# galuszkm/STAN

Hardware: AMD Instinct MI355X
Metric: DOF/s (assembly+CG to 1e-8) on 10M-DOF HEX8 cube; SpMV GB/s vs HBM peak (higher is better)
Workload: dtype f64

## Files before the change

### include/stan_hip.h

```cpp
#ifndef STAN_HIP_H
#define STAN_HIP_H

#include <stdint.h>

#ifdef __cplusplus
extern "C" {
#endif

typedef struct stan_ctx stan_ctx;
typedef struct stan_matrix stan_matrix;

#define STAN_OK 0
#define STAN_E_HIP (-1)
#define STAN_E_ARG (-2)
#define STAN_E_ALLOC (-3)
#define STAN_E_DETJ (-4)
#define STAN_E_DOF_LAYOUT (-5)
#define STAN_E_VALENCE (-6)
#define STAN_E_COMM (-7)
#define STAN_E_UNSUPPORTED (-8)

#define STAN_HEX8_G1 1
#define STAN_HEX8_G2 2

#define STAN_PREC_FP64 0
#define STAN_PREC_MIXED 1
#define STAN_PREC_FIXED48 2
#define STAN_VALUE_STREAM_60 3

int stan_hip_init(int device, stan_ctx **out);
int stan_hip_init_multi(int n_devices, const int *devices, stan_ctx **out);
void stan_hip_destroy(stan_ctx *ctx);
const char *stan_hip_last_error(stan_ctx *ctx);
int64_t stan_hip_last_bad_element(stan_ctx *ctx);
int stan_hip_set_stream(stan_ctx *ctx, void *hip_stream);

#define STAN_OPT_CG_MERIT_STOP 1
#define STAN_OPT_CG_RUPDATE 2
#define STAN_OPT_OVERLAP_HALO 4
#define STAN_OPT_ASSEMBLY_MODE 5
#define STAN_OPT_CG_FUSED_REFRESH 6
#define STAN_OPT_CG_SINGLE_REDUCE 10
#define STAN_OPT_CG_FOLD_REDUCE 11
#define STAN_OPT_VEC_STORE_NT 12
#define STAN_OPT_PACKED_COLUMNS 13
#define STAN_OPT_CG_DEFER_X 14
#define STAN_OPT_SPMV_SMALL 15
#define STAN_OPT_PLACEMENT_TRIES 8
#define STAN_OPT_PLACEMENT_MAX_BYTES 16
#define STAN_OPT_SELL_SIGMA 17
#define STAN_OPT_ROW_FOLDING 19
#define STAN_OPT_COMM_P2P 18
#define STAN_OPT_CG_REFINE 20
#define STAN_OPT_CG_LAZY_SCALING 21
#define STAN_OPT_POOL 7
#define STAN_OPT_POOL_MAX_BYTES 9
#define STAN_OPT_VALUE_STREAM_60 22
#define STAN_OPT_SPMV_VARIANT 3
int stan_hip_set_option(stan_ctx *ctx, int32_t option, int64_t value);
int stan_hip_pool_info(stan_ctx *ctx, int64_t *bytes_parked, int64_t *blocks_parked);

int stan_hip_comm_unique_id(char id[128]);
int stan_hip_comm_init(stan_ctx *ctx, int rank, int nranks, const char id[128]);

int stan_hip_comm_info(stan_ctx *ctx, int32_t *rccl_version, int32_t *comm_ranks, int32_t *comm_rank, int32_t *p2p);
int stan_hip_comm_library(stan_ctx *ctx, char *path, int64_t capacity, int32_t *reused);

int stan_hip_assemble_hex8(stan_ctx *ctx, int64_t n_nodes, const double *xyz,
                           const int32_t *node_dof, int64_t n_elem, const int32_t *conn,
                           const int32_t *elem_mat, const uint8_t *elem_type, int32_t n_mat,
                           const double *mat_E_nu, int64_t n_dof,
                           const int32_t *ndof_reduction, stan_matrix **outK);
int stan_hip_assemble_hex8_dev(stan_ctx *ctx, int64_t n_nodes, const double *d_xyz,
                               const int32_t *d_node_dof, int64_t n_elem, const int32_t *d_conn,
                               const int32_t *d_elem_mat, const uint8_t *d_elem_type,
                               int32_t n_mat, const double *mat_E_nu, int64_t n_dof,
                               const int32_t *d_ndof_reduction, stan_matrix **outK);
void stan_hip_matrix_free(stan_matrix *K);

int stan_hip_cg_solve(stan_ctx *ctx, stan_matrix *K, const double *F, double eps_f,
                      int32_t max_its, int32_t precision_mode, double *U,
                      int32_t *termination_type, int32_t *iterations, double *rel_residual);
int stan_hip_cg_solve_dev(stan_ctx *ctx, stan_matrix *K, const double *d_F, double eps_f,
                          int32_t max_its, int32_t precision_mode, double *d_U,
                          int32_t *termination_type, int32_t *iterations, double *rel_residual);

int stan_hip_cg_solve_multi(stan_ctx *ctx, stan_matrix *K, int32_t n_rhs, const double *F, double eps_f,
                            int32_t max_its, int32_t precision_mode, double *U, int32_t *termination_type,
                            int32_t *iterations, double *rel_residual);
int stan_hip_cg_solve_multi_dev(stan_ctx *ctx, stan_matrix *K, int32_t n_rhs, const double *d_F, double eps_f,
                                int32_t max_its, int32_t precision_mode, double *d_U, int32_t *termination_type,
                                int32_t *iterations, double *rel_residual);

int stan_hip_recover_hex8(stan_ctx *ctx, int64_t n_nodes, const double *xyz, const double *disp,
                          int64_t n_elem, const int32_t *conn, const int32_t *elem_mat,
                          const uint8_t *elem_type, int32_t n_mat, const double *mat_E_nu,
                          double *strain, double *stress);
int stan_hip_recover_hex8_dev(stan_ctx *ctx, int64_t n_nodes, const double *d_xyz,
                              const double *d_disp, int64_t n_elem, const int32_t *d_conn,
                              const int32_t *d_elem_mat, const uint8_t *d_elem_type,
                              int32_t n_mat, const double *mat_E_nu, double *d_strain,
                              double *d_stress);

typedef struct stan_results stan_results;
int stan_hip_recover_hex8_keep(stan_ctx *ctx, int64_t n_nodes, const double *xyz, const double *disp,
                               int64_t n_elem, const int32_t *conn, const int32_t *elem_mat,
                               const uint8_t *elem_type, int32_t n_mat, const double *mat_E_nu, stan_results **out);
int stan_hip_results_map(stan_results *res, int64_t e0, int64_t e1, const double **strain, const double **stress);
void stan_hip_results_free(stan_results *res);

#define STAN_SCALAR_COUNT 24
#define STAN_SCALAR_DISP_X 0
#define STAN_SCALAR_DISP_Y 1
#define STAN_SCALAR_DISP_Z 2
#define STAN_SCALAR_DISP_TOTAL 3
#define STAN_SCALAR_STRESS_XX 4
#define STAN_SCALAR_STRESS_YY 5
#define STAN_SCALAR_STRESS_ZZ 6
#define STAN_SCALAR_STRESS_XY 7
#define STAN_SCALAR_STRESS_YZ 8
#define STAN_SCALAR_STRESS_XZ 9
#define STAN_SCALAR_STRESS_P1 10
#define STAN_SCALAR_STRESS_P2 11
#define STAN_SCALAR_STRESS_P3 12
#define STAN_SCALAR_STRESS_VON_MISES 13
#define STAN_SCALAR_STRAIN_XX 14
#define STAN_SCALAR_STRAIN_YY 15
#define STAN_SCALAR_STRAIN_ZZ 16
#define STAN_SCALAR_STRAIN_XY 17
#define STAN_SCALAR_STRAIN_YZ 18
#define STAN_SCALAR_STRAIN_XZ 19
#define STAN_SCALAR_STRAIN_P1 20
#define STAN_SCALAR_STRAIN_P2 21
#define STAN_SCALAR_STRAIN_P3 22
#define STAN_SCALAR_STRAIN_EFFECTIVE 23
int stan_hip_result_scalars_hex8(stan_ctx *ctx, int64_t n_nodes, const double *disp, int64_t n_elem, const int32_t *conn,
                                 const double *strain, const double *stress, int32_t n_sel, const int32_t *sel,
                                 double *point, double *cell);
int stan_hip_results_scalars(stan_ctx *ctx, stan_results *res, int64_t n_nodes, const double *disp, const int32_t *conn,
                             int32_t n_sel, const int32_t *sel, double *point, double *cell);

int stan_hip_nodal_forces_hex8(stan_ctx *ctx, int64_t n_nodes, const double *xyz, const double *disp,
                               const int32_t *node_dof, int64_t n_elem, const int32_t *conn,
                               const int32_t *elem_mat, const uint8_t *elem_type, int32_t n_mat,
                               const double *mat_E_nu, int64_t n_dof, double *elem_forces, double *R);

typedef struct stan_equilibrium {
    double reaction_sum[3];
    double load_sum[3];
    double fint_sum[3];
    double residual_norm2;
    double load_norm2;
    double residual_max;
    int64_t residual_max_dof;
    int64_t n_fixed;
} stan_equilibrium;
int stan_hip_internal_forces_hex8(stan_ctx *ctx, int64_t n_nodes, const double *xyz, const double *disp,
                                  const int32_t *node_dof, int64_t n_elem, const int32_t *conn,
                                  const int32_t *elem_mat, const uint8_t *elem_type, int32_t n_mat,
                                  const double *mat_E_nu, int64_t n_dof, const int32_t *ndof_reduction,
                                  const double *F, double *f_int, double *reaction, void *eq);
int stan_hip_internal_forces_hex8_dev(stan_ctx *ctx, int64_t n_nodes, const double *d_xyz, const double *d_disp,
                                      const int32_t *d_node_dof, int64_t n_elem, const int32_t *d_conn,
                                      const int32_t *d_elem_mat, const uint8_t *d_elem_type, int32_t n_mat,
                                      const double *mat_E_nu, int64_t n_dof, const int32_t *d_ndof_reduction,
                                      const double *d_F, double *d_f_int, double *d_reaction, void *eq);

typedef struct stan_load_sums {
    double load_sum[3];
    double free_sum[3];
    double volume;
    double area;
    int64_t n_fixed;
    int64_t n_faces;
} stan_load_sums;
int stan_hip_load_vector_hex8(stan_ctx *ctx, int64_t n_nodes, const double *xyz, const int32_t *node_dof,
                              int64_t n_elem, const int32_t *conn, const int32_t *elem_mat, const uint8_t *elem_type,
                              int32_t n_mat, const double *mat_E_nu, int64_t n_dof, const int32_t *ndof_reduction,
                              const double *mat_body, int64_t n_faces, const int32_t *face_elem, const uint8_t *face_id,
                              const double *face_pressure, const double *disp0, double *F, double *F_solve,
                              double *load_full, void *sums);
int stan_hip_load_vector_hex8_dev(stan_ctx *ctx, int64_t n_nodes, const double *d_xyz, const int32_t *d_node_dof,
                                  int64_t n_elem, const int32_t *d_conn, const int32_t *d_elem_mat,
                                  const uint8_t *d_elem_type, int32_t n_mat, const double *mat_E_nu, int64_t n_dof,
                                  const int32_t *d_ndof_reduction, const double *mat_body, int64_t n_faces,
                                  const int32_t *d_face_elem, const uint8_t *d_face_id, const double *d_face_pressure,
                                  const double *d_disp0, double *d_F, double *d_F_solve, double *d_load_full, void *sums);

int stan_hip_load_vector_times(stan_ctx *ctx, double ms[3]);

typedef struct stan_thermal_sums {
    double load_sum[3];
    double free_sum[3];
    double volume;
    double dT_integral;
    int64_t n_fixed;
} stan_thermal_sums;
int stan_hip_thermal_load_hex8(stan_ctx *ctx, int64_t n_nodes, const double *xyz, const int32_t *node_dof,
                               int64_t n_elem, const int32_t *conn, const int32_t *elem_mat, const uint8_t *elem_type,
                               int32_t n_mat, const double *mat_E_nu, int64_t n_dof, const int32_t *ndof_reduction,
                               const double *mat_alpha, const double *dT, double *F, double *load_full, void *sums);
int stan_hip_thermal_load_hex8_dev(stan_ctx *ctx, int64_t n_nodes, const double *d_xyz, const int32_t *d_node_dof,
                                   int64_t n_elem, const int32_t *d_conn, const int32_t *d_elem_mat,
                                   const uint8_t *d_elem_type, int32_t n_mat, const double *mat_E_nu, int64_t n_dof,
                                   const int32_t *d_ndof_reduction, const double *mat_alpha, const double *d_dT, double *d_F,
                                   double *d_load_full, void *sums);
int stan_hip_thermal_stress_hex8(stan_ctx *ctx, int64_t n_nodes, const double *dT, int64_t n_elem, const int32_t *conn,
                                 const int32_t *elem_mat, const uint8_t *elem_type, int32_t n_mat, const double *mat_E_nu,
                                 const double *mat_alpha, double *stress);
int stan_hip_thermal_stress_hex8_dev(stan_ctx *ctx, int64_t n_nodes, const double *d_dT, int64_t n_elem, const int32_t *d_conn,
                                     const int32_t *d_elem_mat, const uint8_t *d_elem_type, int32_t n_mat,
                                     const double *mat_E_nu, const double *mat_alpha, double *d_stress);
int stan_hip_results_thermal_stress(stan_ctx *ctx, stan_results *res, int64_t n_nodes, const double *dT, const int32_t *conn,
// ... 209 lines not shown
```

### stan_amd/csrc/api.hip

```cpp
#include <cstring>

#include "internal.h"

namespace {
thread_local std::string g_err;
}

void stan_set_global_error(const std::string &msg) { g_err = msg; }

extern "C" {

int stan_hip_init(int device, stan_ctx **out) {
    if (!out) return STAN_E_ARG;
    *out = nullptr;
    int n = 0;
    hipError_t e = hipGetDeviceCount(&n);
    if (e != hipSuccess || n <= 0 || device < 0 || device >= n) {
        g_err = std::string("stan_hip_init: no usable HIP device (") +
                (e != hipSuccess ? hipGetErrorString(e) : "device ordinal out of range") + ")";
        return STAN_E_HIP;
    }
    stan_ctx *c = new stan_ctx();
    c->device = device;
    if (hipSetDevice(device) != hipSuccess ||
        hipStreamCreateWithFlags(&c->stream, hipStreamNonBlocking) != hipSuccess ||
        hipHostMalloc((void **)&c->h_status, 64 * sizeof(int64_t), hipHostMallocDefault) != hipSuccess ||
        hipMalloc((void **)&c->d_status, 64 * sizeof(int64_t)) != hipSuccess) {
        g_err = "stan_hip_init: stream / status allocation failed";
        delete c;
        return STAN_E_HIP;
    }
    c->own_stream = true;
    size_t free_b = 0, total_b = 0;
    if (hipMemGetInfo(&free_b, &total_b) == hipSuccess && total_b > 0) c->pool.max_bytes = total_b / 2;
    *out = c;
    return STAN_OK;
}

void stan_hip_destroy(stan_ctx *ctx) {
    if (!ctx) return;
    if (ctx->group) { stan_group_destroy(ctx); return; }
    hipSetDevice(ctx->device);
    if (ctx->p2p && ctx->p2p->ipc) stan_p2p_ipc_release(ctx);
    {
        void *comm = nullptr;
        { std::lock_guard<std::mutex> lk(ctx->comm_mu); comm = ctx->comm; ctx->comm = nullptr; }
        if (comm && ctx->nccl.CommDestroy) ctx->nccl.CommDestroy(comm);
    }
    if (ctx->own_stream && ctx->stream) hipStreamDestroy(ctx->stream);
    if (ctx->side) hipStreamDestroy(ctx->side);
    if (ctx->ev_a) hipEventDestroy(ctx->ev_a);
    if (ctx->ev_b) hipEventDestroy(ctx->ev_b);
    for (stan_matrix *K : ctx->matrices) K->ctx = nullptr;
    stan_cg_workspace_free(ctx);
    ctx->pool.flush();
    if (ctx->h_status) hipHostFree(ctx->h_status);
    if (ctx->d_status) hipFree(ctx->d_status);
    delete ctx;
}

const char *stan_hip_last_error(stan_ctx *ctx) {
    if (ctx && ctx->group) return stan_group_last_error(ctx);
    return ctx ? ctx->err.c_str() : g_err.c_str();
}
int64_t stan_hip_last_bad_element(stan_ctx *ctx) { return ctx ? ctx->bad_elem : -1; }

int stan_hip_set_stream(stan_ctx *ctx, void *hip_stream) {
    if (!ctx) return STAN_E_ARG;
    STAN_NO_GROUP(ctx, "set_stream");
    hipSetDevice(ctx->device);
    if (ctx->stream) hipStreamSynchronize(ctx->stream);
    if (ctx->own_stream && ctx->stream) hipStreamDestroy(ctx->stream);
    ctx->own_stream = false;
    ctx->stream = (hipStream_t)hip_stream;
    if (!hip_stream) {
        HIPCHK(ctx, hipStreamCreateWithFlags(&ctx->stream, hipStreamNonBlocking));
        ctx->own_stream = true;
    }
    return STAN_OK;
}

int stan_hip_set_option(stan_ctx *ctx, int32_t option, int64_t value) {
    if (!ctx) return STAN_E_ARG;
    if (ctx->group && option == STAN_OPT_COMM_P2P) return stan_group_set_p2p(ctx, value != 0);
    if (ctx->group)
        return stan_group_ctx_call(ctx, [&](stan_ctx *c) { return stan_hip_set_option(c, option, value); });
    if (option == STAN_OPT_COMM_P2P) {
        if (value != 0) {
            if (ctx->nranks < 2 || !ctx->comm) { ctx->err = "STAN_OPT_COMM_P2P: needs a communicator of several ranks (stan_hip_comm_init) or a handle of stan_hip_init_multi"; return STAN_E_UNSUPPORTED; }
            HIPCHK(ctx, hipSetDevice(ctx->device));
            STANCHK(stan_p2p_ipc_setup(ctx));
        }
        ctx->comm_p2p = value != 0 && ctx->p2p != nullptr;
        return STAN_OK;
    }
    if (option == STAN_OPT_CG_MERIT_STOP) ctx->cg_merit_stop = value != 0;
    else if (option == STAN_OPT_CG_RUPDATE && value >= 0 && value < (1 << 30)) ctx->cg_rupdate = (int)value;
    else if (option == STAN_OPT_ASSEMBLY_MODE && (value == 0 || value == 1)) ctx->assembly_mode = (int)value;
    else if (option == STAN_OPT_CG_FUSED_REFRESH) ctx->cg_fused_refresh = value != 0;
    else if (option == STAN_OPT_CG_SINGLE_REDUCE) ctx->cg_single_reduce = value != 0;
    else if (option == STAN_OPT_CG_FOLD_REDUCE) ctx->cg_fold_reduce = value != 0;
    else if (option == STAN_OPT_CG_REFINE && value >= 0 && value <= 2) ctx->cg_refine = (int)value;
    else if (option == STAN_OPT_CG_LAZY_SCALING) ctx->cg_lazy_scaling = value != 0;
    else if (option == STAN_OPT_VEC_STORE_NT && value >= 0 && value <= 3) ctx->vec_store_nt = (int)value;
    else if (option == STAN_OPT_PACKED_COLUMNS) ctx->cols16 = value != 0;
    else if (option == STAN_OPT_CG_DEFER_X) ctx->cg_defer_x = value != 0;
    else if (option == STAN_OPT_SPMV_SMALL && value >= 0) ctx->spmv_small_rows = value == 1 ? 150000 : value;
    else if (option == STAN_OPT_POOL) {
        ctx->pool.enabled = value != 0;
        if (!ctx->pool.enabled) {
            hipSetDevice(ctx->device);
            hipStreamSynchronize(ctx->stream);
            ctx->pool.flush();
        }
    }
    else if (option == STAN_OPT_POOL_MAX_BYTES && value >= -1) {
        hipSetDevice(ctx->device);
        if (value == -1) {
            size_t free_b = 0, total_b = 0;
            if (hipMemGetInfo(&free_b, &total_b) != hipSuccess) { (void)hipGetLastError(); ctx->err = "set_option: hipMemGetInfo failed"; return STAN_E_HIP; }
            value = (int64_t)(free_b - free_b / 10 + ctx->pool.bytes_avail);
        }
        ctx->pool.max_bytes = (size_t)value;
        hipStreamSynchronize(ctx->stream);
        while (!ctx->pool.avail.empty() && ctx->pool.bytes_avail > ctx->pool.max_bytes) {
            hipFree(ctx->pool.avail.front().p);
            ctx->pool.bytes_avail -= ctx->pool.avail.front().cap;
            ctx->pool.avail.erase(ctx->pool.avail.begin());
        }
    }
    else if (option == STAN_OPT_VALUE_STREAM_60 && value >= -1 && value <= 1) ctx->value_stream_60 = (int)value;
    else if (option == STAN_OPT_OVERLAP_HALO) ctx->overlap_halo = value != 0;
    else if (option == STAN_OPT_SELL_SIGMA && value >= 1 && value <= 32) ctx->sell_sigma = (int)value;
    else if (option == STAN_OPT_PLACEMENT_TRIES && value >= 1 && value <= 64) ctx->placement_tries = (int)value;
    else if (option == STAN_OPT_PLACEMENT_MAX_BYTES && value >= 0) ctx->placement_max_bytes = value;
    else if (option == STAN_OPT_ROW_FOLDING && value >= -1 && value <= 1) ctx->row_folding = (int)value;
    else if (option == STAN_OPT_SPMV_VARIANT && (value == -1 || value == 0 || value == 9 || value == 12 || value == 20))
        ctx->spmv_variant = (int)value;
    else { ctx->err = "set_option: unknown option or bad value"; return STAN_E_ARG; }
    return STAN_OK;
}

int stan_hip_pool_info(stan_ctx *ctx, int64_t *bytes_parked, int64_t *blocks_parked) {
    if (!ctx) return STAN_E_ARG;
    if (ctx->group) ctx = stan_group_rank0(ctx);
    if (bytes_parked) *bytes_parked = (int64_t)ctx->pool.bytes_avail;
    if (blocks_parked) *blocks_parked = (int64_t)ctx->pool.avail.size();
    return STAN_OK;
}

int stan_hip_comm_info(stan_ctx *ctx, int32_t *rccl_version, int32_t *comm_ranks, int32_t *comm_rank, int32_t *p2p) {
    if (!ctx) return STAN_E_ARG;
    stan_ctx *c = ctx->group ? stan_group_rank0(ctx) : ctx;
    int v = 0, n = 0, r = 0;
    stan_comm_info(c, &v, &n, &r);
    if (rccl_version) *rccl_version = v;
    if (comm_ranks) *comm_ranks = n;
    if (comm_rank) *comm_rank = r;
    if (p2p) *p2p = (c->p2p && c->comm_p2p) ? 1 : 0;
    return STAN_OK;
}

int stan_hip_comm_library(stan_ctx *ctx, char *path, int64_t capacity, int32_t *reused) {
    if (!ctx || (capacity > 0 && !path) || capacity < 0) return STAN_E_ARG;
    stan_ctx *c = ctx->group ? stan_group_rank0(ctx) : ctx;
    std::string p;
    int r = 0;
    stan_comm_library(c, &p, &r);
    if (capacity > 0) {
        const size_t n = p.size() < (size_t)capacity - 1 ? p.size() : (size_t)capacity - 1;
        memcpy(path, p.data(), n);
        path[n] = 0;
    }
    if (reused) *reused = r;
    return STAN_OK;
}

int stan_hip_set_profiling(stan_ctx *ctx, int32_t enabled) {
    if (!ctx) return STAN_E_ARG;
    if (ctx->group)
        return stan_group_ctx_call(ctx, [&](stan_ctx *c) { return stan_hip_set_profiling(c, enabled); });
    ctx->profiling = enabled != 0;
    return STAN_OK;
}
int stan_hip_get_profile_rank(stan_ctx *ctx, int32_t rank, stan_profile *out) {
    if (!ctx || !out || rank < 0) return STAN_E_ARG;
    if (ctx->group) {
        if (rank >= stan_group_size(ctx)) return STAN_E_ARG;
        return stan_hip_get_profile(stan_group_rank(ctx, rank), out);
    }
    if (rank != 0) return STAN_E_ARG;
    return stan_hip_get_profile(ctx, out);
}
int stan_hip_device_info(stan_ctx *ctx, int32_t rank, int32_t *hip_ordinal, char bus_id[32]) {
    if (!ctx || rank < 0) return STAN_E_ARG;
    stan_ctx *c = ctx;
    if (ctx->group) {
        if (rank >= stan_group_size(ctx)) return STAN_E_ARG;
        c = stan_group_rank(ctx, rank);
    } else if (rank != 0) return STAN_E_ARG;
    if (hip_ordinal) *hip_ordinal = c->device;
    if (bus_id) {
        bus_id[0] = 0;
        if (hipDeviceGetPCIBusId(bus_id, 32, c->device) != hipSuccess) { (void)hipGetLastError(); bus_id[0] = 0; }
    }
    return STAN_OK;
}
int stan_hip_get_profile(stan_ctx *ctx, stan_profile *out) {
    if (!ctx || !out) return STAN_E_ARG;
    if (ctx->group) ctx = stan_group_rank0(ctx);
    *out = ctx->prof;
    out->assembly_colours = ctx->prof_colours;
    out->placement_candidates = ctx->prof_placement_candidates;
    out->placement_ms_best = ctx->prof_placement_ms_best;
    out->placement_ms_worst = ctx->prof_placement_ms_worst;
    out->placement_moved_vectors = ctx->prof_placement_moved_vectors;
    return STAN_OK;
}

}
```

### stan_amd/csrc/cg.hip

```cpp
#include <chrono>
#include <cmath>
#include <thread>
#include <type_traits>
#include <utility>

#include "internal.h"
#include "s60.h"
#include "p2p_device.h"
#include "fx48.h"


namespace {

#include "cg_reduce_device.inc"

#include "cg_setup_kernels.inc"

#include "spmv_kernels.inc"

#include "cg_vector_kernels.inc"

#include "cg_multi.inc"

inline unsigned vec_grid(int64_t n) {
    int64_t b = (n + VEC_T - 1) / VEC_T;
    if (b < 1) b = 1;
    return (unsigned)(b > VEC_BLOCKS ? VEC_BLOCKS : b);
}

inline void launch_reduce(hipStream_t stream, int nv, const double *partial, int np, double *out, p2p_out po, const int64_t *st, int64_t k) {
    if (nv == 2) hipLaunchKernelGGL(k_reduce<2>, dim3(1), dim3(256), 0, stream, partial, np, out, po, st, k);
    else hipLaunchKernelGGL(k_reduce<1>, dim3(1), dim3(256), 0, stream, partial, np, out, po, st, k);
}

struct span_list {
    const stan_ctx *ctx;
    event_bag *bag;
    std::vector<hipEvent_t> ev;
    std::vector<int64_t> its;
    void mark(hipStream_t s) { ev.push_back(bag->make()); hipEventRecord(ev.back(), s); }
    void begin(hipStream_t s, int64_t k = 0) { if (ctx->profiling) { mark(s); its.push_back(k); } }
    void end(hipStream_t s) { if (ctx->profiling) mark(s); }
    void drain(int64_t max_k, double *ms, int64_t *n) {
        for (size_t i = 0; i + 1 < ev.size(); i += 2) {
            float t = 0;
            if (its[i / 2] <= max_k && hipEventElapsedTime(&t, ev[i], ev[i + 1]) == hipSuccess) { *ms += t; (*n)++; }
        }
        ev.clear(); its.clear();
    }
};

struct chunk_poll {
    static constexpr int64_t hard_cap = 0x7fffffff;
    hipEvent_t ev[2] = {nullptr, nullptr};
    int64_t *slot[2] = {nullptr, nullptr};
    int chunk_id = 0;
    void setup(event_bag &events, int64_t *pinned, size_t stride) {
        for (int i = 0; i < 2; i++) { ev[i] = events.make(hipEventDisableTiming); slot[i] = pinned + stride * i; }
    }
    template <typename WAIT, typename STOPPED>
    int poll(stan_ctx *ctx, hipStream_t st, const int64_t *status, size_t words, int64_t k, WAIT wait, STOPPED stopped, bool *done) {
        HIPCHK(ctx, hipMemcpyAsync(slot[chunk_id & 1], status, words * 8, hipMemcpyDeviceToHost, st));
        HIPCHK(ctx, hipEventRecord(ev[chunk_id & 1], st));
        if (chunk_id > 0) {
            STANCHK(wait(ev[(chunk_id - 1) & 1]));
            if (stopped(slot[(chunk_id - 1) & 1])) *done = true;
        }
        if (k >= hard_cap) *done = true;
        chunk_id++;
        return STAN_OK;
    }
};

constexpr int64_t STREAM60_AUTO_ROWS = 150000;

struct product_plan {
    enum { SMALL, PAIR, WAVE } form = WAVE;
    int forced_var = -1;
    bool folding = false;
    int spb = 4;
    unsigned blocks = 0;
    int vs = STAN_PREC_FP64;
    bool may_lazy_scale = false;
    bool stream60 = false;
    bool folded = false;
    const stan_colpack *cols = nullptr;
    int64_t slots = 0;
    int var(bool fx) const { return forced_var >= 0 ? forced_var : fx ? 12 : 9; }
    void fold_planned(const stan_matrix *K) { may_lazy_scale = may_lazy_scale && !(folding && K->fold_state == 1); }
    void value_stream_built(const stan_matrix *K) { if (vs == STAN_PREC_FIXED48 && !K->vs[vs].padded) vs = STAN_PREC_FP64; }
    void copies_built(const stan_matrix *K) {
        stream60 = stream60 && !K->vs[STAN_VALUE_STREAM_60].refused && !(folding && K->fold_state == 1);
        folded = folding && K->vs[vs].folded != nullptr;
        cols = folded ? &K->fold_pk : &K->pk;
        slots = folded ? K->nfslots : K->nslots;
    }
    void stream60_unavailable() { stream60 = false; }
};

product_plan plan_products(const stan_ctx *ctx, const stan_matrix *K, int precision_mode, bool dist, bool sr) {
    product_plan P;
    const int v = ctx->spmv_variant;
    P.form = v < 0 && K->nb_glob <= ctx->spmv_small_rows ? product_plan::SMALL : v == 20 ? product_plan::PAIR : product_plan::WAVE;
    P.forced_var = v;
    P.folding = ctx->row_folding != 0;
    P.spb = P.form == product_plan::SMALL ? 1 : P.form == product_plan::PAIR ? 2 : 4;
    P.blocks = nblk(K->nslices, P.spb);
    P.vs = precision_mode;
    const bool fp64_one_rank = precision_mode == STAN_PREC_FP64 && !dist && P.form != product_plan::SMALL && K->nslices > 0;
    P.may_lazy_scale = !K->scaled && ctx->cg_lazy_scaling && fp64_one_rank && v < 0 && ctx->cg_rupdate != 1;
    P.stream60 = ctx->value_stream_60 != 0 && fp64_one_rank && !sr && (v < 0 || v == 9 || v == 12) &&
                 (ctx->value_stream_60 > 0 || K->nb_glob > STREAM60_AUTO_ROWS);
    return P;
}

inline colstream colstream_of(const stan_ctx *ctx, const stan_colpack &c, int64_t nslots) {
    return ctx->cols16 && c.cols16 ? make_colstream(c, nslots) : NO_COLSTREAM;
}

struct product_args {
    const double *x;
    double *y;
    const double *x2;
    double *y2;
    int dot;
    double *partial;
    const int64_t *st;
    int64_t k;
    int kind;
    const void *vals;
    bool vals_folded;
    bool first;
};
template <typename F>
void with_product_types(const stan_matrix *K, const product_args &a, F f) {
    auto by_dot = [&](auto *vals) {
        if (a.dot == 2) f(vals, std::integral_constant<int, 2>());
        else if (a.dot == 1) f(vals, std::integral_constant<int, 1>());
        else f(vals, std::integral_constant<int, 0>());
    };
    const void *vals = a.vals ? a.vals : K->vs[a.kind].padded;
    if (a.kind == STAN_PREC_MIXED) by_dot((const float *)vals);
    else if (a.kind == STAN_PREC_FIXED48) by_dot((const uint32_t *)vals);
    else by_dot((const double *)vals);
}
template <typename VT>
const VT *fold_vals(const product_plan &P, const stan_matrix *K, const product_args &a, const VT *vals) {
    if (a.vals_folded) return vals;
    const stan_value_stream &s = K->vs[a.kind];
    return P.folding && (const void *)vals == s.padded ? (const VT *)s.folded : nullptr;
}
unsigned launch_product(stan_ctx *ctx, stan_matrix *K, const product_plan &P, const product_args &a, int which = 0,
                        hipStream_t stream = nullptr, fold_args fold = NO_FOLD) {
    if (!stream) stream = ctx->stream;
    const int32_t *slist = which == 1 ? K->d_sl_int : which == 2 ? K->d_sl_bnd : nullptr;
    const int32_t nlist = which == 1 ? K->n_sl_int : which == 2 ? K->n_sl_bnd : K->nslices;
    const bool s60 = a.kind == STAN_VALUE_STREAM_60;
    const bool plain = !a.x2 && !a.first && !s60, small = plain && P.form == product_plan::SMALL, pair = plain && P.form == product_plan::PAIR;
    const int spb = plain ? P.spb : 4;
    const int32_t poff = which == 2 ? (int32_t)nblk(K->n_sl_int, spb) : 0;
    const unsigned grid = nblk(nlist, spb);
    if (grid == 0) return 0;
    fold.nblocks = grid;
    fold.np = (int)grid + poff;
    const colstream cs = colstream_of(ctx, K->pk, K->nslots);
    if (s60) {
        const s60_t *vals = (const s60_t *)(a.vals ? a.vals : K->vs[a.kind].padded);
        auto launch = [&](auto var) {
            hipLaunchKernelGGL((k_spmv<s60_t, 1, decltype(var)::value>), dim3(grid), dim3(256), 0, stream, K->nslices, K->nloc, K->d_slot_ptr,
                               K->d_rowof, K->d_cols, vals, a.x, a.y, a.partial, a.st, a.k, slist, nlist, poff, fold, cs);
        };
        if (P.var(false) == 12) launch(std::integral_constant<int, 12>());
        else launch(std::integral_constant<int, 9>());
        return grid;
    }
    with_product_types(K, a, [&](auto *vals, auto dot_tag) {
        using VT = std::remove_cv_t<std::remove_pointer_t<decltype(vals)>>;
        constexpr int DOT = decltype(dot_tag)::value;
        const dim3 g(grid), b(256);
        const VT *fv = small || pair || a.first ? nullptr : fold_vals(P, K, a, vals);
        const colstream fcs = colstream_of(ctx, K->fold_pk, K->nfslots);
        if constexpr (std::is_same_v<VT, double>)
            if (a.first) {
                hipLaunchKernelGGL(k_spmv_first<DOT>, g, b, 0, stream, K->nslices, K->nloc, K->d_slot_ptr, K->d_rowof, K->d_cols,
                                   K->vals64(), K->d_scale, a.x, a.y, a.partial, a.st, a.k, fold, cs);
                return;
            }
        if constexpr (DOT == 1)
            if (a.x2) {
                if (fv)
                    hipLaunchKernelGGL((k_spmv_fold<VT, 1, 2>), g, b, 0, stream, K->nslices, K->nloc, K->d_fold_ptr, K->d_rowof,
                                       K->d_fold_meta, K->d_fold_cols, fv, a.x, a.x2, a.y, a.y2, a.partial, a.st, a.k, slist, nlist,
                                       poff, fold, fcs);
                else
                    hipLaunchKernelGGL((k_spmv2<VT>), g, b, 0, stream, K->nslices, K->nloc, K->d_slot_ptr, K->d_rowof, K->d_cols,
                                       vals, a.x, a.x2, a.y, a.y2, a.partial, a.st, a.k, slist, nlist, poff, fold, cs);
                return;
            }
        if (small) {
            hipLaunchKernelGGL((k_spmv_small<VT, DOT>), g, b, 0, stream, K->nslices, K->nloc, K->d_slot_ptr, K->d_rowof,
                               K->d_cols, vals, a.x, a.y, a.partial, a.st, a.k, slist, nlist, poff, fold, cs);
            return;
        }
        if (pair) {
            hipLaunchKernelGGL((k_spmv_pair<VT, DOT, true>), g, b, 0, stream, K->nslices, K->nloc, K->d_slot_ptr, K->d_rowof,
                               K->d_cols, vals, a.x, a.y, a.partial, a.st, a.k, slist, nlist, poff, fold, cs);
            return;
        }
        if (fv) {
            hipLaunchKernelGGL((k_spmv_fold<VT, DOT, 1>), g, b, 0, stream, K->nslices, K->nloc, K->d_fold_ptr, K->d_rowof,
                               K->d_fold_meta, K->d_fold_cols, fv, a.x, (const double *)nullptr, a.y, (double *)nullptr, a.partial,
                               a.st, a.k, slist, nlist, poff, fold, fcs);
            return;
        }
#define SPMV_CASE(V)                                                                                                          \
    case V:                                                                                                                   \
        hipLaunchKernelGGL((k_spmv<VT, DOT, V>), g, b, 0, stream, K->nslices, K->nloc, K->d_slot_ptr, K->d_rowof, K->d_cols, \
                           vals, a.x, a.y, a.partial, a.st, a.k, slist, nlist, poff, fold, cs);                               \
        break;
        switch (P.var(vstream<VT>::FX)) {
            SPMV_CASE(9) SPMV_CASE(12)
            default:
            SPMV_CASE(0)
        }
#undef SPMV_CASE
    });
    return grid;
}

}

static int ensure_scale_vector(stan_ctx *ctx, stan_matrix *K) {
    const int64_t npad = (int64_t)K->nslices * 64;
    const int64_t ns = 3 * (npad + K->nhalo);
    if (!K->d_scale) STANCHK(stan_dmalloc(ctx, &K->d_scale, (size_t)ns));
    hipLaunchKernelGGL(k_fill, dim3(vec_grid(ns)), dim3(VEC_T), 0, ctx->stream, K->d_scale, ns, 1.0);
    if (K->nloc > 0)
        hipLaunchKernelGGL(k_diag_scale, dim3(nblk(K->nloc, 256)), dim3(256), 0, ctx->stream, K->nloc,
                           K->d_rowlen, K->d_posof, K->d_slot_ptr, K->d_cols, K->vals64(), K->d_scale);
    if (stan_sharded(ctx)) {
        if (ctx->comm_p2p && ctx->p2p) {
            const p2p_out po{stan_p2p_table(ctx), stan_p2p_reduce_slot(ctx), 3, 1};
            launch_reduce(ctx->stream, 1, nullptr, 0, nullptr, po, nullptr, 0);
            STANCHK(stan_p2p_reduce_wait(ctx));
        }
        STANCHK(stan_comm_halo_exchange(ctx, K, K->d_scale));
    }
    HIPCHK(ctx, hipGetLastError());
    return STAN_OK;
}
static void mark_scaled(stan_ctx *ctx, stan_matrix *K) {
    K->scaled = true;
    for (int kind = STAN_PREC_FP64 + 1; kind < STAN_NSTREAMS; kind++) {
        stan_dfree(ctx, K->vs[kind].padded);
        K->vs[kind].padded = nullptr;
        K->vs[kind].refused = false;
    }
    stan_matrix_drop_folded_values(ctx, K);
}
static int ensure_scaled(stan_ctx *ctx, stan_matrix *K) {
    if (K->scaled) return STAN_OK;
    STANCHK(ensure_scale_vector(ctx, K));
    if (K->nslices > 0)
        hipLaunchKernelGGL(k_scale_matrix, dim3(nblk(K->nslices, 4)), dim3(256), 0, ctx->stream,
                           K->nslices, K->d_slot_ptr, K->d_rowof, K->d_cols, K->vals64(), K->d_scale);
    HIPCHK(ctx, hipGetLastError());
    mark_scaled(ctx, K);
    return STAN_OK;
}

int stan_matrix_ensure_scaled(stan_ctx *ctx, stan_matrix *K) { return ensure_scaled(ctx, K); }

static int cg_wait(stan_ctx *ctx, bool p2p, hipStream_t st, hipEvent_t ev) {
    if (!p2p) {
        if (ev) HIPCHK(ctx, hipEventSynchronize(ev));
        else HIPCHK(ctx, hipStreamSynchronize(st));
        return STAN_OK;
    }
    const double bound = stan_p2p_stall_seconds();
    const auto t0 = std::chrono::steady_clock::now();
    int spins = 0;
    for (;;) {
        const hipError_t e = ev ? hipEventQuery(ev) : hipStreamQuery(st);
        if (e == hipSuccess) return STAN_OK;
        if (e != hipErrorNotReady) { ctx->err = std::string("cg: ") + hipGetErrorString(e); (void)hipGetLastError(); return STAN_E_HIP; }
        (void)hipGetLastError();
        if (++spins > 200) std::this_thread::sleep_for(std::chrono::microseconds(spins > 2000 ? 500 : 50));
        if (ctx->p2p->broken.load()) break;
        if (std::chrono::duration<double>(std::chrono::steady_clock::now() - t0).count() > bound) break;
    }
    stan_p2p_release_own(ctx);
    (void)hipStreamSynchronize(st);
    (void)hipGetLastError();
    ctx->err = "cg: peer-to-peer exchange made no progress (a peer rank failed or never arrived); this rank's waits were released";
    return STAN_E_COMM;
}

namespace {

struct cg_run {
    stan_ctx *ctx;
    stan_matrix *K;
    const double *d_F;
    double eps_f;
    int32_t max_its;
    int32_t precision_mode;
    double *d_U;

    hipStream_t st_ = nullptr;
    event_bag events;
    hipEvent_t ev0 = nullptr, ev1 = nullptr;
    bool dist = false, p2p = false, sr = false, foldr = false, split = false;
    product_plan plan;
    bool lazy_scale = false;
    bool reduced = false;
    uint32_t *pend60 = nullptr;
    int64_t n60 = 0;
    ~cg_run() { if (pend60) stan_dfree(ctx, pend60); }
    int refine = 0;
    int64_t n3 = 0, npad = 0, ng = 0, dof0 = 0;
    dev_scope bufs{ctx};
    double *xb[2] = {nullptr, nullptr}, *p = nullptr, *r = nullptr, *v = nullptr, *w = nullptr, *bh = nullptr;
    double *partial = nullptr, *sc = nullptr, *sv = nullptr;
    double *xacc = nullptr, *b0 = nullptr;
    int64_t *stt = nullptr;
    unsigned long long *tick = nullptr;
    const stan_p2p_dev *p2p_tab = nullptr;
    unsigned vg = 1;
    int64_t its_before_restart = 1;
    int64_t *h_st = nullptr;
    double *h_sc = nullptr;
    chunk_poll poll;
    span_list red_sp{ctx, &events}, halo_sp{ctx, &events}, spmv_sp{ctx, &events}, spmv2_sp{ctx, &events}, spmv64_sp{ctx, &events};
    int64_t n_coll = 0, n_wait = 0, n_launch = 0, n_enqueued = 0;
    double prof_spmv_ms = 0, prof_spmv2_ms = 0, prof_spmv64_ms = 0;
    int64_t prof_spmv_n = 0, prof_spmv2_n = 0, prof_spmv64_n = 0;
    int pass_type = 0;
    int64_t pass_its = 0;
    const double *xfin = nullptr;

    p2p_out p2p_to(int j0, bool signal) {
        return p2p ? p2p_out{p2p_tab, stan_p2p_reduce_slot(ctx), j0, signal ? 1 : 0} : NO_P2P;
    }
    fold_args fold_to(int which, double *out, p2p_out po = NO_P2P) {
        return fold_args{foldr ? tick + FOLD_WORDS * which : nullptr, 0, 0, out, po};
    }
    fold_args vec_fold(double *out, p2p_out po = NO_P2P) {
        fold_args f = fold_to(1, out, po);
        f.nblocks = vg; f.np = (int)vg;
        return f;
    }
    void reduce_if_unfolded(int np, int nv, double *out, p2p_out po = NO_P2P, int64_t k_ = -1) {
        if (foldr || np <= 0) return;
        const int64_t *sk = k_ >= 1 ? stt : nullptr;
        launch_reduce(st_, nv, partial, np, out, po, sk, k_);
    }
    int exchange_sums(double *scalars, int count, red_src *rs) {
        *rs = red_src{nullptr, 0, nullptr, 0};
        if (!dist) return STAN_OK;
        red_sp.begin(st_);
        int rc_ = STAN_OK;
        if (p2p) {
            *rs = red_src{stan_p2p_mailbox(ctx, stan_p2p_reduce_slot(ctx)), ctx->nranks, nullptr, 0};
            rc_ = stan_p2p_reduce_wait(ctx, &rs->ctr, &rs->want);
            if (!rs->ctr) n_wait++;
        } else {
            rc_ = stan_comm_allreduce_sum_f64(ctx, scalars, (size_t)count);
            n_coll++;
        }
        red_sp.end(st_);
        return rc_;
    }
    int halo(double *x) {
        halo_sp.begin(st_);
        const int rc_ = stan_comm_halo_exchange(ctx, K, x);
        if (p2p && !K->nbr.empty()) n_wait++;
        halo_sp.end(st_);
        return rc_;
    }

    int product(double *x, double *x2, double *y, int dot, double *out, int64_t k, p2p_out po, int kind, bool extra = false) {
        span_list &span = extra ? spmv64_sp : x2 ? spmv2_sp : spmv_sp;
        if (pend60 && K->scaled) {
            const int rc = stan_matrix_encode_s60(ctx, K, std::exchange(pend60, nullptr));
            if (!K->vs[STAN_VALUE_STREAM_60].padded) plan.stream60_unavailable();
            STANCHK(rc);
        }
        const bool s60 = plan.stream60 && !pend60 && !x2 && dot == 1 && !extra && !lazy_scale && kind == STAN_PREC_FP64;
        if (s60) { kind = STAN_VALUE_STREAM_60; n60++; }
        span.begin(st_, k);
        auto go = [&](int which, hipStream_t s, bool last) -> unsigned {
            n_launch++;
            const product_args a{x, y, x2, x2 ? w : nullptr, dot, partial, stt, k, kind, nullptr, false, lazy_scale};
            const unsigned blocks = launch_product(ctx, K, plan, a, which, s, (dot && last) ? fold_to(0, out, po) : NO_FOLD);
            if (lazy_scale) { lazy_scale = false; mark_scaled(ctx, K); }
            return blocks;
        };
        unsigned parts = 0;
        bool folded = foldr;
        if (split) {
            HIPCHK(ctx, hipEventRecord(ctx->ev_a, st_));
            HIPCHK(ctx, hipStreamWaitEvent(ctx->side, ctx->ev_a, 0));
            parts = go(1, ctx->side, false);
            HIPCHK(ctx, hipEventRecord(ctx->ev_b, ctx->side));
            STANCHK(halo(x));
            if (x2) STANCHK(halo(x2));
            HIPCHK(ctx, hipStreamWaitEvent(st_, ctx->ev_b, 0));
            const unsigned pb = go(2, st_, true);
            if (pb == 0) folded = false;
            parts += pb;
        } else {
            if (dist) { STANCHK(halo(x)); if (x2) STANCHK(halo(x2)); }
            parts = go(0, st_, true);
            if (parts == 0) folded = false;
        }
        if (dot && !folded) {
            if (parts > 0 || po.pp) {
                launch_reduce(st_, dot, partial, (int)parts, out, po, k >= 1 ? stt : nullptr, k);
                n_launch++;
            } else HIPCHK(ctx, hipMemsetAsync(out, 0, 8 * dot, st_));
        }
        span.end(st_);
        return STAN_OK;
    }

    int setup();
    int begin_pass(bool from_F, double eps_pass, bool *done);
    int iterate(double eps_pass, int32_t max_its_pass);
    int pass(bool from_F, double eps_pass, int32_t max_its_pass);
    void account_pass();
    int fp64_check(double *xg, const double *b, double *r2_out);
    int finish(const double *x_result, int type, int64_t its, double rel_rec, double rel64, int passes,
               int32_t *term_out, int32_t *iters_out, double *rel_res_out);
};

int cg_run::setup() {
    st_ = ctx->stream;
    if (ctx->profiling) {
        ev0 = events.make(); ev1 = events.make();
        hipEventRecord(ev0, st_);
    }
    dist = stan_sharded(ctx);
    p2p = dist && ctx->comm_p2p && ctx->p2p != nullptr;
    if (p2p && ctx->p2p->broken.load()) {
        ctx->err = "cg: the peer-to-peer exchange of this context is broken (a peer rank failed earlier); start a fresh process";
        return STAN_E_COMM;
    }
    if (p2p || (dist && ctx->peers_share_device)) ctx->defer_frees = true;
    STANCHK(stan_cg_workspace(ctx, K));
    if (p2p) {
        const int64_t ns_ = 3 * ((int64_t)K->nslices * 64 + K->nhalo);
        if (!K->d_scale) STANCHK(stan_dmalloc(ctx, &K->d_scale, (size_t)ns_));
        double *const pub[5] = {ctx->ws.xb[0], ctx->ws.xb[1], ctx->ws.p, ctx->ws.r, K->d_scale};
        STANCHK(stan_p2p_publish_vectors(ctx, K, pub));
    }
    sr = ctx->cg_single_reduce;
    foldr = ctx->cg_fold_reduce;
    plan = plan_products(ctx, K, precision_mode, dist, sr);
    auto folded_copy = [&](int kind, bool plan_only) {
        const int rc = stan_matrix_make_folded(ctx, K, kind, plan_only);
        if (rc == STAN_E_ALLOC) { stan_matrix_abandon_folding(ctx, K); ctx->err.clear(); }
        return rc == STAN_E_ALLOC ? (int)STAN_OK : rc;
    };
    if (plan.may_lazy_scale) {
        STANCHK(folded_copy(STAN_PREC_FP64, true));
        plan.fold_planned(K);
    }
    lazy_scale = plan.may_lazy_scale;
    if (lazy_scale) STANCHK(ensure_scale_vector(ctx, K));
    else STANCHK(ensure_scaled(ctx, K));
    if (ctx->cols16) STANCHK(stan_matrix_make_cols16(ctx, K));
    if (precision_mode == STAN_PREC_MIXED) STANCHK(stan_matrix_make_fp32(ctx, K));
    if (precision_mode == STAN_PREC_FIXED48) STANCHK(stan_matrix_make_fx48(ctx, K));
    reduced = precision_mode != STAN_PREC_FP64;
    refine = reduced ? ctx->cg_refine : 0;
    plan.value_stream_built(K);
    if (plan.form != product_plan::SMALL) STANCHK(folded_copy(plan.vs, false));
    plan.copies_built(K);
    if (plan.stream60 && !K->vs[STAN_VALUE_STREAM_60].padded) {
        STANCHK(stan_matrix_alloc_s60(ctx, K, &pend60));
        if (!pend60) plan.stream60_unavailable();
    }

    n3 = 3 * K->nloc;
    npad = (int64_t)K->nslices * 64;
    ng = gather_len(K);
    dof0 = 3 * K->r0;
    xb[0] = ctx->ws.xb[0]; xb[1] = ctx->ws.xb[1]; p = ctx->ws.p; r = ctx->ws.r;
    v = ctx->ws.v; w = ctx->ws.w; bh = ctx->ws.bh;
    if (sr) sv = ctx->ws.sv;
    const size_t npart = 2 * (size_t)(plan.blocks > VEC_BLOCKS ? plan.blocks : VEC_BLOCKS) + 16;
    STANCHK(bufs.alloc(&partial, npart));
    STANCHK(bufs.alloc(&sc, (size_t)S_NSCAL));
    STANCHK(bufs.alloc(&stt, (size_t)T_NSTAT));
    STANCHK(bufs.alloc(&tick, (size_t)(2 * FOLD_WORDS)));
    HIPCHK(ctx, hipMemsetAsync(sc, 0, S_NSCAL * 8, st_));
    HIPCHK(ctx, hipMemsetAsync(tick, 0, 2 * FOLD_WORDS * 8, st_));
    HIPCHK(ctx, hipMemsetAsync(xb[0], 0, (size_t)ng * 8, st_));
    HIPCHK(ctx, hipMemsetAsync(xb[1], 0, (size_t)ng * 8, st_));
    HIPCHK(ctx, hipMemsetAsync(p, 0, (size_t)ng * 8, st_));
    if (sr) {
        HIPCHK(ctx, hipMemsetAsync(r, 0, (size_t)ng * 8, st_));
        HIPCHK(ctx, hipMemsetAsync(sv, 0, (size_t)n3 * 8, st_));
    }
    p2p_tab = p2p ? stan_p2p_table(ctx) : nullptr;
    vg = vec_grid(n3);
    its_before_restart = K->n_red > 0 ? K->n_red : 1;
    split = dist && ctx->overlap_halo && K->d_sl_bnd != nullptr;
    if (split && !ctx->side) {
        HIPCHK(ctx, hipStreamCreateWithFlags(&ctx->side, hipStreamNonBlocking));
        HIPCHK(ctx, hipEventCreateWithFlags(&ctx->ev_a, hipEventDisableTiming));
        HIPCHK(ctx, hipEventCreateWithFlags(&ctx->ev_b, hipEventDisableTiming));
    }
    h_st = ctx->h_status + SS_H_CG_STATUS;
    h_sc = (double *)(ctx->h_status + SS_H_CG_SCALARS);
    poll.setup(events, h_st, 8);
    return STAN_OK;
}

int cg_run::begin_pass(bool from_F, double eps_pass, bool *done) {
    {
        const fold_args f = vec_fold(sc + S_VMV, p2p_to(0, true));
        if (from_F)
            hipLaunchKernelGGL(k_init, dim3(vg), dim3(VEC_T), 0, st_, n3, dof0, K->d_red, d_F, K->d_scale,
                               bh, xb[0], r, p, partial, f);
        else
            hipLaunchKernelGGL(k_init_b, dim3(vg), dim3(VEC_T), 0, st_, n3, (const double *)r, bh, xb[0], r, p, partial, f);
        reduce_if_unfolded((int)vg, 1, sc + S_VMV, p2p_to(0, true));
    }
    red_src rs_b;
    STANCHK(exchange_sums(sc + S_VMV, 1, &rs_b));
    hipLaunchKernelGGL(k_init_scalars, dim3(1), dim3(64), 0, st_, sc, stt, eps_pass, rs_b);
    HIPCHK(ctx, hipGetLastError());
    HIPCHK(ctx, hipMemcpyAsync(h_st, stt, T_NSTAT * 8, hipMemcpyDeviceToHost, st_));
    STANCHK(cg_wait(ctx, p2p, st_, nullptr));
    *done = h_st[T_ITER_A] == 0;
    return STAN_OK;
}

int cg_run::iterate(double eps_pass, int32_t max_its_pass) {
    int64_t k = 1;
    bool done = false;
    int rc = STAN_OK;
    poll.chunk_id = 0;
    red_src rs_sr{nullptr, 0, nullptr, 0}, rs_vmv{nullptr, 0, nullptr, 0}, rs_r2{nullptr, 0, nullptr, 0};
    const bool refresh64 = refine >= 2;
    const int kind_refresh = refresh64 ? STAN_PREC_FP64 : plan.vs;
    constexpr int REFRESH64 = 50;
    const int rupdate = refresh64 ? (ctx->cg_rupdate > 0 ? REFRESH64 : 0) : ctx->cg_rupdate;
    if (sr) {
        if (p2p)
            launch_reduce(st_, 1, partial, 0, sc + S_SR_MERIT, p2p_to(2, false), nullptr, 0);
        rc = product(r, nullptr, w, 2, sc + S_SR_GAMMA, 0, p2p_to(0, true), plan.vs);
        if (rc == STAN_OK) rc = exchange_sums(sc + S_SR_GAMMA, 3, &rs_sr);
    }
    const int chunk = dist ? CHUNK_DIST : CHUNK;
    while (!done && rc == STAN_OK) {
        for (int c = 0; c < chunk && k < chunk_poll::hard_cap; c++, k++) {
            const bool refresh = rupdate > 0 && (k % rupdate) == 0;
            if (sr) {
                sr_args a;
                a.n3 = n3; a.k = k; a.sc = sc; a.st = stt; a.epsf = eps_pass; a.maxits = max_its_pass;
                a.its_before_restart = its_before_restart; a.merit_stop = ctx->cg_merit_stop ? 1 : 0;
                a.refresh = refresh ? 1 : 0;
                a.xcur = xb[(k - 1) & 1]; a.xnext = xb[k & 1];
                a.r = r; a.p = p; a.s = sv; a.w = w; a.bh = bh; a.partial = partial;
                a.rs = rs_sr;
                a.fold = vec_fold(sc + S_SR_MERIT, p2p_to(2, false));
                hipLaunchKernelGGL(k_vec_sr, dim3(vg), dim3(VEC_T), 0, st_, a);
                n_launch++;
                if (!refresh) reduce_if_unfolded((int)vg, 1, sc + S_SR_MERIT, p2p_to(2, false), k);
                else {
                    rc = product(xb[k & 1], nullptr, v, 0, nullptr, k, NO_P2P, kind_refresh, refresh64);
                    if (rc) break;
                    hipLaunchKernelGGL(k_refresh, dim3(vg), dim3(VEC_T), 0, st_, n3, k, (const int64_t *)stt,
                                       bh, v, xb[k & 1], r, partial, vec_fold(sc + S_SR_DELTA, p2p_to(1, false)));
                    n_launch++;
                    reduce_if_unfolded((int)vg, 2, sc + S_SR_DELTA, p2p_to(1, false), k);
                }
                rc = product(r, nullptr, w, 2, sc + S_SR_GAMMA, k, p2p_to(0, true), plan.vs);
                if (rc) break;
                rc = exchange_sums(sc + S_SR_GAMMA, 3, &rs_sr);
                if (rc) break;
                continue;
            }
            const bool fused = refresh && ctx->cg_fused_refresh && !refresh64;
            rc = product(p, fused ? xb[(k - 1) & 1] : nullptr, v, 1, sc + S_VMV, k, p2p_to(0, true), plan.vs);
            if (rc) break;
            rc = exchange_sums(sc + S_VMV, 1, &rs_vmv);
            if (rc) break;
            const p2p_out po_r = p2p_to(0, true);
            step_args a;
            a.rs_vmv = rs_vmv;
            a.n3 = n3; a.k = k; a.sc = sc; a.st = stt;
            a.xcur = xb[(k - 1) & 1]; a.xnext = xb[k & 1];
            a.r = r; a.p = p; a.v = v; a.w = w; a.bh = bh; a.partial = partial;
            a.refresh = refresh ? (fused ? 2 : 1) : 0;
            a.merit = ctx->cg_merit_stop ? 1 : 0;
            a.defer_x = (ctx->cg_defer_x && !a.merit && a.refresh != 1) ? 1 : 0;
            a.fold = vec_fold(sc + S_R2NEW, a.refresh == 1 ? NO_P2P : po_r);
            hipLaunchKernelGGL((ctx->vec_store_nt & 2) ? k_step<true> : k_step<false>, dim3(vg), dim3(VEC_T), 0, st_, a);
            n_launch++;
            if (a.refresh == 1) {
                rc = product(xb[k & 1], nullptr, v, 0, nullptr, k, NO_P2P, kind_refresh, refresh64);
                if (rc) break;
                hipLaunchKernelGGL(k_refresh, dim3(vg), dim3(VEC_T), 0, st_, n3, k,
                                   (const int64_t *)stt, bh, v, xb[k & 1], r, partial, vec_fold(sc + S_R2NEW, po_r));
                n_launch++;
            }
            if (!foldr) { reduce_if_unfolded((int)vg, 2, sc + S_R2NEW, po_r, k); n_launch++; }
            rc = exchange_sums(sc + S_R2NEW, 2, &rs_r2);
            if (rc) break;
            const double *ux = a.defer_x ? a.xcur : nullptr;
            double *uxn = a.defer_x ? a.xnext : nullptr;
            hipLaunchKernelGGL((ctx->vec_store_nt & 1) ? k_update<true> : k_update<false>, dim3(vg), dim3(VEC_T), 0, st_, n3, k, sc, stt,
                               eps_pass, (int64_t)max_its_pass, its_before_restart, ctx->cg_merit_stop ? 1 : 0, r, p, ux, uxn, rs_r2, rs_vmv);
            n_launch++;
        }
        if (rc) break;
        STANCHK(poll.poll(ctx, st_, stt, T_NSTAT, k, [&](hipEvent_t e) { return cg_wait(ctx, p2p, st_, e); },
                          [](const int64_t *w) { return w[T_TYPE] != 0; }, &done));
        if (dist && (ctx->comm_broken.load() || (ctx->p2p && ctx->p2p->broken.load()))) {
            ctx->err = "cg: a peer rank failed (the exchanges were aborted)";
            rc = STAN_E_COMM;
        }
    }
    n_enqueued += k - 1;
    if (p2p) {
        if (rc == STAN_OK) rc = cg_wait(ctx, true, st_, nullptr);
        else stan_p2p_release_own(ctx);
    }
    hipError_t e = hipStreamSynchronize(st_);
    if (rc) return rc;
    if (e != hipSuccess) { ctx->err = std::string("cg: ") + hipGetErrorString(e); return STAN_E_HIP; }
    HIPCHK(ctx, hipMemcpyAsync(h_st, stt, T_NSTAT * 8, hipMemcpyDeviceToHost, st_));
    HIPCHK(ctx, hipMemcpyAsync(h_sc, sc, S_NSCAL * 8, hipMemcpyDeviceToHost, st_));
    HIPCHK(ctx, hipStreamSynchronize(st_));
    pass_type = (int)h_st[T_TYPE];
    pass_its = h_st[T_ITERS];
    if (pass_type == 0) { pass_type = 5; pass_its = k - 1; h_st[T_XSEL] = (k - 1) & 1; }
    xfin = xb[h_st[T_XSEL] & 1];
    return STAN_OK;
}

int cg_run::pass(bool from_F, double eps_pass, int32_t max_its_pass) {
    bool done = false;
    STANCHK(begin_pass(from_F, eps_pass, &done));
    if (done) {
        HIPCHK(ctx, hipMemcpyAsync(h_sc, sc, S_NSCAL * 8, hipMemcpyDeviceToHost, st_));
        HIPCHK(ctx, hipStreamSynchronize(st_));
        pass_type = (int)h_st[T_TYPE];
        pass_its = h_st[T_ITERS];
        xfin = xb[h_st[T_XSEL] & 1];
        return STAN_OK;
    }
    STANCHK(iterate(eps_pass, max_its_pass));
    account_pass();
    return STAN_OK;
}

void cg_run::account_pass() {
    spmv_sp.drain(pass_its, &prof_spmv_ms, &prof_spmv_n);
    spmv2_sp.drain(pass_its, &prof_spmv2_ms, &prof_spmv2_n);
}

int cg_run::fp64_check(double *xg, const double *b, double *r2_out) {
    STANCHK(product(xg, nullptr, v, 0, nullptr, 0, NO_P2P, STAN_PREC_FP64, true));
    const p2p_out po = p2p_to(0, true);
    hipLaunchKernelGGL(k_refresh, dim3(vg), dim3(VEC_T), 0, st_, n3, (int64_t)0, (const int64_t *)stt, b, v,
                       (const double *)xg, r, partial, vec_fold(sc + S_CHK_R2, po));
    n_launch++;
    reduce_if_unfolded((int)vg, 2, sc + S_CHK_R2, po);
    red_src rs;
    STANCHK(exchange_sums(sc + S_CHK_R2, 2, &rs));
    if (rs.mb) hipLaunchKernelGGL(k_land_sums, dim3(1), dim3(64), 0, st_, sc + S_CHK_R2, rs);
    HIPCHK(ctx, hipGetLastError());
    HIPCHK(ctx, hipMemcpyAsync(h_sc, sc, S_NSCAL * 8, hipMemcpyDeviceToHost, st_));
    STANCHK(cg_wait(ctx, p2p, st_, nullptr));
    *r2_out = h_sc[S_CHK_R2];
    spmv64_sp.drain(chunk_poll::hard_cap, &prof_spmv64_ms, &prof_spmv64_n);
    return STAN_OK;
}

int cg_run::finish(const double *x_result, int type, int64_t its, double rel_rec, double rel64, int passes,
                   int32_t *term_out, int32_t *iters_out, double *rel_res_out) {
    if (!dist || ctx->result_segment) {
        hipLaunchKernelGGL(k_result, dim3(vg), dim3(VEC_T), 0, st_, n3, dof0, K->d_red, K->d_scale,
                           x_result, d_U);
    } else {
        double *full;
        STANCHK(bufs.alloc(&full, (size_t)K->n_dof));
        hipLaunchKernelGGL(k_result_full, dim3(vg), dim3(VEC_T), 0, st_, n3, K->d_scale, x_result,
                           full + dof0);
        STANCHK(stan_comm_allgather_rows(ctx, K, full));
        hipLaunchKernelGGL(k_compress, dim3(vec_grid(K->n_dof)), dim3(VEC_T), 0, st_, K->n_dof,
                           K->d_red, full, d_U);
    }
    HIPCHK(ctx, hipGetLastError());
    if (ctx->profiling) hipEventRecord(ev1, st_);
    HIPCHK(ctx, hipStreamSynchronize(st_));

    if (term_out) *term_out = type;
    if (iters_out) *iters_out = (int32_t)(its > chunk_poll::hard_cap ? chunk_poll::hard_cap : its);
    if (rel_res_out) *rel_res_out = rel64 >= 0 ? rel64 : rel_rec;
    if (!ctx->profiling) return STAN_OK;
    float ms = 0;
    hipEventElapsedTime(&ms, ev0, ev1);
    stan_profile &pf = ctx->prof;
    pf.cg_ms = ms;
    pf.spmv_ms_total = prof_spmv_ms;
    pf.spmv_launches = prof_spmv_n;
    pf.spmv2_ms_total = prof_spmv2_ms;
    pf.spmv2_launches = prof_spmv2_n;
    pf.fp64_products = (int32_t)prof_spmv64_n;
    pf.fp64_products_ms = prof_spmv64_ms;
    pf.iterations = (int32_t)its;
    pf.termination_type = type;
    pf.rel_residual_recurrence = rel_rec;
    pf.rel_residual_fp64 = rel64;
    pf.refine_passes = passes;
    const int stream = n60 > 0 ? (int)STAN_VALUE_STREAM_60 : plan.vs;
    const stan_colpack &c = *plan.cols;
    const bool read_packed = ctx->cols16 && c.cols16;
    const double packed_frac = read_packed && plan.slots > 0 ? (double)c.slots_packed / (double)plan.slots : 0.0;
    pf.spmv_bytes = K->nblocks * (4 * K->vs[stream].dwords + 4) + 3 * K->nloc * 16 + K->nloc * (plan.folded ? 8 : 4)
                    - (int64_t)(packed_frac * (double)K->nblocks * 2.0) + (read_packed ? (c.slots_packed + c.slots_packed2) * 4 : 0);
    pf.repacked_streams = plan.folded ? 1 : 0;
    pf.col_slots_packed = ctx->cols16 && K->pk.cols16 ? K->pk.slots_packed : 0;
    pf.value_stream = stream;
    pf.cg_iteration_vector_bytes = 3 * K->nloc * 8 * ((ctx->cg_defer_x && !ctx->cg_merit_stop ? 8 : 9) + (ctx->cg_merit_stop ? 1 : 0));
    pf.loop_kernel_launches = n_launch;
    pf.loop_collectives = n_coll;
    pf.loop_stream_waits = n_wait;
    pf.loop_iterations_enqueued = n_enqueued;
    pf.comm_reduce_ms_total = pf.comm_halo_ms_total = 0;
    pf.comm_reduce_calls = pf.comm_halo_calls = 0;
    red_sp.drain(chunk_poll::hard_cap, &pf.comm_reduce_ms_total, &pf.comm_reduce_calls);
    halo_sp.drain(chunk_poll::hard_cap, &pf.comm_halo_ms_total, &pf.comm_halo_calls);
    return STAN_OK;
}

}

int stan_cg_device(stan_ctx *ctx, stan_matrix *K, const double *d_F, double eps_f,
                   int32_t max_its, int32_t precision_mode, double *d_U, int32_t *term_out,
                   int32_t *iters_out, double *rel_res_out) {
    if (precision_mode != STAN_PREC_FP64 && precision_mode != STAN_PREC_MIXED &&
        precision_mode != STAN_PREC_FIXED48) {
        ctx->err = "cg_solve: unknown precision_mode";
        return STAN_E_UNSUPPORTED;
    }
    if (eps_f < 0 || max_its < 0) {
        ctx->err = "cg_solve: eps_f and max_its must be >= 0";
        return STAN_E_ARG;
    }
    if (eps_f == 0 && max_its == 0) eps_f = 1.0e-6;
    struct free_later { stan_ctx *c; ~free_later() { if (c->defer_frees) { stan_flush_deferred(c); stan_p2p_ipc_trim(c); } } } free_guard{ctx};
    cg_run R{ctx, K, d_F, eps_f, max_its, precision_mode, d_U};
    STANCHK(R.setup());

    constexpr int MAX_PASSES = 8;
    int type = 0, passes = 0;
    int64_t its = 0;
    double bnorm0 = 0, rel_rec = 0, rel64 = -1.0, prev_rel64 = 0, eps_pass = eps_f;
    const double *x_result = nullptr;
    for (;;) {
        const int64_t left = max_its > 0 ? (int64_t)max_its - its : 0;
        STANCHK(R.pass(passes == 0, eps_pass, (int32_t)left));
        passes++;
        its += R.pass_its;
        type = R.pass_type;
        if (passes == 1) bnorm0 = R.h_sc[S_BNORM];
        rel_rec = bnorm0 > 0 ? std::sqrt(R.h_sc[S_R2OUT]) / bnorm0 : 0.0;
        x_result = R.xfin;
        if (!R.reduced) break;
        double *xg = const_cast<double *>(R.xfin);
        if (passes > 1) {
            hipLaunchKernelGGL(k_accumulate, dim3(R.vg), dim3(VEC_T), 0, R.st_, R.n3, R.xacc, R.xfin, R.p);
            xg = R.p;
            x_result = R.xacc;
        }
        double r2 = 0;
        STANCHK(R.fp64_check(xg, passes > 1 ? R.b0 : R.bh, &r2));
        rel64 = bnorm0 > 0 ? std::sqrt(r2) / bnorm0 : 0.0;
        const bool met = rel64 <= eps_f || bnorm0 == 0;
        if (type != 1) break;
        if (met) break;
        const bool out_of_its = max_its > 0 && its >= max_its;
        const bool stalled = passes > 1 && !(rel64 < 0.5 * prev_rel64);
        if (R.refine == 0 || passes >= MAX_PASSES || out_of_its || stalled || !std::isfinite(rel64)) {
            type = out_of_its ? 5 : 7;
            break;
        }
        if (passes == 1) {
            STANCHK(R.bufs.alloc(&R.xacc, (size_t)(R.n3 > 0 ? R.n3 : 1)));
            STANCHK(R.bufs.alloc(&R.b0, (size_t)(R.n3 > 0 ? R.n3 : 1)));
            HIPCHK(ctx, hipMemcpyAsync(R.xacc, R.xfin, (size_t)R.n3 * 8, hipMemcpyDeviceToDevice, R.st_));
            HIPCHK(ctx, hipMemcpyAsync(R.b0, R.bh, (size_t)R.n3 * 8, hipMemcpyDeviceToDevice, R.st_));
        }
        prev_rel64 = rel64;
        eps_pass = eps_f / rel64;
        HIPCHK(ctx, hipMemsetAsync(R.sc, 0, S_NSCAL * 8, R.st_));
        if (R.sr) HIPCHK(ctx, hipMemsetAsync(R.sv, 0, (size_t)R.n3 * 8, R.st_));
    }
    return R.finish(x_result, type, its, rel_rec, rel64, passes, term_out, iters_out, rel_res_out);
}

namespace {

constexpr int MULTI_MAX = 8;

struct pinned_words {
    int64_t *p = nullptr;
    ~pinned_words() { if (p) (void)hipHostFree(p); }
};

struct cg_multi_run {
    stan_ctx *ctx;
    stan_matrix *K;
    double eps_f;
    int32_t max_its;
    hipStream_t st_ = nullptr;
    dev_scope bufs{ctx};
    int64_t n3 = 0, ng = 0, pstride = 0, its_before_restart = 1;
    unsigned vg = 1, pg = 0;
    double *xb[2] = {nullptr, nullptr}, *p = nullptr, *r = nullptr, *v = nullptr, *bh = nullptr, *partial = nullptr, *sc = nullptr;
    int64_t *stt = nullptr;
    unsigned long long *tick = nullptr;
    pinned_words host;
    event_bag events;
    chunk_poll poll;

    int setup(int mmax) {
        st_ = ctx->stream;
        STANCHK(ensure_scaled(ctx, K));
        if (ctx->cols16) STANCHK(stan_matrix_make_cols16(ctx, K));
        n3 = 3 * K->nloc;
        ng = gather_len(K);
        vg = vec_grid(n3);
        pg = nblk(K->nslices, 4);
        pstride = 2 * (int64_t)(pg > VEC_BLOCKS ? pg : VEC_BLOCKS) + 16;
        its_before_restart = K->n_red > 0 ? K->n_red : 1;
        const size_t m = (size_t)mmax, g = (size_t)(ng > 0 ? ng : 1), n = (size_t)(n3 > 0 ? n3 : 1);
        for (double **q : {&xb[0], &xb[1], &p}) STANCHK(bufs.alloc(q, g * m));
        for (double **q : {&r, &v, &bh}) STANCHK(bufs.alloc(q, n * m));
        STANCHK(bufs.alloc(&partial, (size_t)pstride * m));
        STANCHK(bufs.alloc(&sc, (size_t)S_NSCAL * m));
        STANCHK(bufs.alloc(&stt, (size_t)T_NSTAT * m));
        STANCHK(bufs.alloc(&tick, (size_t)(2 * FOLD_WORDS)));
        HIPCHK(ctx, hipHostMalloc((void **)&host.p, (size_t)(3 * T_NSTAT + S_NSCAL) * MULTI_MAX * 8, hipHostMallocDefault));
        poll.setup(events, host.p, MULTI_MAX * T_NSTAT);
        return STAN_OK;
    }

    template <int M>
    int group(const double *d_F, double *d_U, int32_t *term_out, int32_t *iters_out, double *rel_out) {
        const int64_t nr = K->n_red;
        const size_t g = (size_t)(ng > 0 ? ng : 1);
        const int merit = ctx->cg_merit_stop ? 1 : 0, rupdate = ctx->cg_rupdate;
        const colstream cs = colstream_of(ctx, K->pk, K->nslots);
        const fold_args fvec{tick + FOLD_WORDS, vg, (int)vg, nullptr, NO_P2P};
        const fold_args fprod{tick, pg, (int)pg, nullptr, NO_P2P};
        int64_t *h_st = host.p + 2 * MULTI_MAX * T_NSTAT;
        double *h_sc = (double *)(host.p + 3 * MULTI_MAX * T_NSTAT);
        HIPCHK(ctx, hipMemsetAsync(sc, 0, (size_t)S_NSCAL * M * 8, st_));
        HIPCHK(ctx, hipMemsetAsync(stt, 0, (size_t)T_NSTAT * M * 8, st_));
        HIPCHK(ctx, hipMemsetAsync(tick, 0, 2 * FOLD_WORDS * 8, st_));
        for (double *q : {xb[0], xb[1], p}) HIPCHK(ctx, hipMemsetAsync(q, 0, g * M * 8, st_));
        hipLaunchKernelGGL(k_init_m<M>, dim3(vg), dim3(VEC_T), 0, st_, n3, nr, K->d_red, d_F, K->d_scale, bh, xb[0], r, p, partial,
                           pstride, sc, fvec);
        hipLaunchKernelGGL(k_init_scalars_m<M>, dim3(1), dim3(64), 0, st_, sc, stt, eps_f);
        HIPCHK(ctx, hipGetLastError());
        HIPCHK(ctx, hipMemcpyAsync(h_st, stt, (size_t)T_NSTAT * M * 8, hipMemcpyDeviceToHost, st_));
        HIPCHK(ctx, hipStreamSynchronize(st_));
        auto all_stopped = [&](const int64_t *w) {
            for (int c = 0; c < M; c++) if (w[c * T_NSTAT + T_TYPE] == 0) return false;
            return true;
        };
        bool done = all_stopped(h_st) || pg == 0;
        int64_t k = 1;
        poll.chunk_id = 0;
        while (!done) {
            for (int c = 0; c < CHUNK && k < chunk_poll::hard_cap; c++, k++) {
// ... 90 lines not shown
```

### stan_amd/csrc/cg_reduce_device.inc

```

constexpr int VEC_BLOCKS = 2048;
constexpr int VEC_T = 256;
constexpr int CHUNK = 32;
constexpr int CHUNK_DIST = 8;

enum { S_BNORM = 0, S_VMV = 1, S_R2NEW = 2, S_MERIT = 3, S_RHO0 = 4, S_RHO1 = 5, S_PMF0 = 6,
       S_PMF1 = 7, S_R2OUT = 8,
       S_SR_GAMMA = 9, S_SR_DELTA = 10, S_SR_MERIT = 11, S_SR_GP0 = 12, S_SR_GP1 = 13, S_SR_AP0 = 14,
       S_SR_AP1 = 15,
       S_CHK_R2 = 16, S_CHK_MF = 17, S_NSCAL = 24 };
enum { T_ITER_A = 0, T_ITER_B = 1, T_TYPE = 2, T_ITERS = 3, T_XSEL = 4, T_NSTAT = 8 };

__device__ __forceinline__ double wave_sum(double v) {
#pragma unroll
    for (int d = 32; d > 0; d >>= 1) v += __shfl_xor(v, d, 64);
    return v;
}
__device__ __forceinline__ double block_sum(double v, double *sh) {
    v = wave_sum(v);
    const int lane = threadIdx.x & 63, w = threadIdx.x >> 6;
    __syncthreads();
    if (lane == 0) sh[w] = v;
    __syncthreads();
    return sh[0] + sh[1] + sh[2] + sh[3];
}

__device__ __forceinline__ void st_agent(double *p, double v) {
    __hip_atomic_store(p, v, __ATOMIC_RELAXED, __HIP_MEMORY_SCOPE_AGENT);
}
__device__ __forceinline__ double ld_agent(const double *p) {
    return __hip_atomic_load(p, __ATOMIC_RELAXED, __HIP_MEMORY_SCOPE_AGENT);
}
template <int NV>
__device__ __forceinline__ void sum_partials(const double *partial, int np, double *sh, double r[NV]) {
    constexpr int W = 16 / NV;
    double a[NV][W];
#pragma unroll
    for (int j = 0; j < NV; j++)
#pragma unroll
        for (int q = 0; q < W; q++) a[j][q] = 0;
    int i = threadIdx.x;
    for (; i + (W - 1) * 256 < np; i += W * 256) {
#pragma unroll
        for (int q = 0; q < W; q++)
#pragma unroll
            for (int j = 0; j < NV; j++) a[j][q] += ld_agent(partial + (int64_t)(i + q * 256) * NV + j);
    }
    for (; i < np; i += 256)
#pragma unroll
        for (int j = 0; j < NV; j++) a[j][0] += ld_agent(partial + (int64_t)i * NV + j);
#pragma unroll
    for (int j = 0; j < NV; j++) {
#pragma unroll
        for (int w = W / 2; w > 0; w >>= 1)
#pragma unroll
            for (int q = 0; q < w; q++) a[j][q] += a[j][q + w];
        r[j] = block_sum(a[j][0], sh);
    }
}
constexpr int FOLD_SUB = 32;
constexpr int FOLD_LINE = 16;
constexpr int FOLD_WORDS = (1 + FOLD_SUB) * FOLD_LINE;
struct fold_args {
    unsigned long long *counter;
    unsigned nblocks;
    int np;
    double *out;
    p2p_out po;
};
constexpr p2p_out NO_P2P = {nullptr, 0, 0, 0};
constexpr fold_args NO_FOLD = {nullptr, 0, 0, nullptr, NO_P2P};
template <int NV>
__device__ __forceinline__ void publish_sums(double *out, const p2p_out &po, const double r[NV], double *sh) {
    if (po.pp) { p2p_publish<NV>(po, r, sh); return; }
    if (threadIdx.x == 0) {
#pragma unroll
        for (int j = 0; j < NV; j++) out[j] = r[j];
    }
}
__device__ __forceinline__ bool fold_arrive(const fold_args &f, int *sh_last) {
    if (threadIdx.x == 0) {
        asm volatile("s_waitcnt vmcnt(0)" ::: "memory");
        const unsigned sub = blockIdx.x % FOLD_SUB;
        const unsigned in_sub = (f.nblocks - sub + FOLD_SUB - 1) / FOLD_SUB;
        const unsigned nsub = f.nblocks < (unsigned)FOLD_SUB ? f.nblocks : (unsigned)FOLD_SUB;
        int last = 0;
        unsigned long long t = __hip_atomic_fetch_add(f.counter + (1 + sub) * FOLD_LINE, 1ULL, __ATOMIC_RELAXED,
                                                      __HIP_MEMORY_SCOPE_AGENT);
        if (t == (unsigned long long)in_sub - 1) {
            t = __hip_atomic_fetch_add(f.counter, 1ULL, __ATOMIC_RELAXED, __HIP_MEMORY_SCOPE_AGENT);
            last = t == (unsigned long long)nsub - 1;
        }
        *sh_last = last;
    }
    __syncthreads();
    return *sh_last != 0;
}
template <int NV>
__device__ __forceinline__ void fold_finish(const fold_args &f, const double *partial, double *sh) {
    double r[NV];
    sum_partials<NV>(partial, f.np, sh, r);
    publish_sums<NV>(f.out, f.po, r, sh);
    if (threadIdx.x <= FOLD_SUB)
        __hip_atomic_store(f.counter + threadIdx.x * FOLD_LINE, 0ULL, __ATOMIC_RELAXED, __HIP_MEMORY_SCOPE_AGENT);
}

__device__ __forceinline__ void fold_skip(const fold_args &f) {
    if (f.counter && f.po.pp && f.po.signal && blockIdx.x == 0 && (int)threadIdx.x < f.po.pp->n)
        __hip_atomic_fetch_add(f.po.pp->sig_red[threadIdx.x][f.po.slot], 1ULL, __ATOMIC_RELAXED, __HIP_MEMORY_SCOPE_SYSTEM);
}

__device__ __forceinline__ bool stopped(const int64_t *st, int64_t k) {
    return st[T_ITER_A] < k || st[T_ITER_B] < k;
}
```

### stan_amd/csrc/cg_vector_kernels.inc

```

__device__ __forceinline__ double vld_ro(const double *q) {
    return __builtin_nontemporal_load(q);
}
__device__ __forceinline__ double vld_rmw(const double *q) {
    return __builtin_nontemporal_load(q);
}

struct step_args {
    int64_t n3;
    int64_t k;
    double *sc;
    int64_t *st;
    const double *xcur;
    double *xnext;
    double *r;
    const double *p;
    const double *v;
    const double *bh;
    double *partial;
    const double *w;
    int merit;
    int refresh;
    int defer_x;
    fold_args fold;
    red_src rs_vmv;
};

template <bool RNT>
__global__ void __launch_bounds__(VEC_T) k_step(step_args a) {
    __shared__ double sh[4];
    __shared__ int sh_last;
    if (stopped(a.st, a.k)) { if (a.refresh != 1) fold_skip(a.fold); return; }
    double vmv_[1];
    red_get<1>(a.sc + S_VMV, a.rs_vmv, vmv_, sh);
    const double vmv = vmv_[0];
    const double rho = a.sc[S_RHO0 + (a.k & 1)];
    int bad = 0;
    if (!isfinite(vmv) || vmv <= 0) bad = isfinite(vmv) ? -5 : -4;
    const double alpha = rho / vmv;
    if (!bad && !isfinite(alpha)) bad = -4;
    if (bad) {
        if (blockIdx.x == 0 && threadIdx.x == 0) {
            a.st[T_TYPE] = bad;
            a.st[T_ITERS] = a.k;
            a.st[T_XSEL] = (a.k - 1) & 1;
            a.st[T_ITER_B] = a.k;
        }
        if (a.refresh != 1) fold_skip(a.fold);
        return;
    }
    double s_r2 = 0, s_mf = 0;
    const int64_t stride = (int64_t)gridDim.x * VEC_T;
    for (int64_t i = (int64_t)blockIdx.x * VEC_T + threadIdx.x; i < a.n3; i += stride) {
        double cx = 0;
        if (!a.defer_x) {
            const double pi = __builtin_nontemporal_load(a.p + i);
            cx = __builtin_nontemporal_load(a.xcur + i) + alpha * pi;
            __builtin_nontemporal_store(cx, a.xnext + i);
        }
        if (a.refresh == 0) {
            const double cr = vld_rmw(a.r + i) - alpha * vld_ro(a.v + i);
            if (RNT) __builtin_nontemporal_store(cr, a.r + i);
            else a.r[i] = cr;
            s_r2 += cr * cr;
            if (a.merit) s_mf -= (cr + a.bh[i]) * cx;
        } else if (a.refresh == 2) {
            const double b = a.bh[i];
            const double mv = a.w[i] + alpha * a.v[i];
            const double cr = b - mv;
            if (RNT) __builtin_nontemporal_store(cr, a.r + i);
            else a.r[i] = cr;
            s_r2 += cr * cr;
            if (a.merit) s_mf += (mv - 2 * b) * cx;
        }
    }
    if (a.refresh != 1) {
        const double t0 = block_sum(s_r2, sh);
        const double t1 = block_sum(s_mf, sh);
        if (threadIdx.x == 0) {
            st_agent(a.partial + 2 * blockIdx.x, t0);
            st_agent(a.partial + 2 * blockIdx.x + 1, t1);
        }
        if (a.fold.counter && fold_arrive(a.fold, &sh_last)) fold_finish<2>(a.fold, a.partial, sh);
    }
}

__global__ void __launch_bounds__(VEC_T)
k_refresh(int64_t n3, int64_t k, const int64_t *st, const double *bh, const double *mv,
          const double *cx, double *r, double *partial, fold_args fold) {
    __shared__ double sh[4];
    __shared__ int sh_last;
    if (st[T_ITER_A] < k || st[T_ITER_B] <= k) { fold_skip(fold); return; }
    double s_r2 = 0, s_mf = 0;
    const int64_t stride = (int64_t)gridDim.x * VEC_T;
    for (int64_t i = (int64_t)blockIdx.x * VEC_T + threadIdx.x; i < n3; i += stride) {
        const double b = bh[i], m = mv[i];
        const double cr = b - m;
        __builtin_nontemporal_store(cr, r + i);
        s_r2 += cr * cr;
        s_mf += (m - 2 * b) * cx[i];
    }
    const double t0 = block_sum(s_r2, sh);
    const double t1 = block_sum(s_mf, sh);
    if (threadIdx.x == 0) {
        st_agent(partial + 2 * blockIdx.x, t0);
        st_agent(partial + 2 * blockIdx.x + 1, t1);
    }
    if (fold.counter && fold_arrive(fold, &sh_last)) fold_finish<2>(fold, partial, sh);
}

template <bool PNT>
__global__ void __launch_bounds__(VEC_T)
k_update(int64_t n3, int64_t k, double *sc, int64_t *st, double epsf, int64_t maxits,
         int64_t its_before_restart, int merit_stop, const double *r, double *p,
         const double *xcur, double *xnext ,
         red_src rs_r2, red_src rs_vmv) {
    __shared__ double sh[4];
    if (st[T_ITER_A] < k || st[T_ITER_B] <= k) return;
    double t2[2];
    red_get<2>(sc + S_R2NEW, rs_r2, t2, sh);
    const double r2 = t2[0], merit = t2[1];
    const double rho = sc[S_RHO0 + (k & 1)], prevmf = sc[S_PMF0 + (k & 1)];
    const double bnorm = sc[S_BNORM];
    int type = 0;
    int64_t xsel = k & 1;
    if (sqrt(r2) <= epsf * bnorm) type = 1;
    else if (k >= maxits && maxits > 0) type = 5;
    else if (merit_stop && merit >= prevmf) { type = 7; xsel = (k - 1) & 1; }
    double beta = 0;
    const bool restart = (k % its_before_restart) == 0;
    if (!type && !restart) {
        beta = r2 / rho;
        if (!isfinite(beta)) { type = -4; }
    }
    if (blockIdx.x == 0 && threadIdx.x == 0) {
        sc[S_R2OUT] = r2;
        if (type) {
            st[T_TYPE] = type;
            st[T_ITERS] = k;
            st[T_XSEL] = xsel;
            st[T_ITER_A] = k;
        } else {
            sc[S_RHO0 + ((k + 1) & 1)] = r2;
            sc[S_PMF0 + ((k + 1) & 1)] = merit;
        }
    }
    const int64_t stride = (int64_t)gridDim.x * VEC_T;
    double alpha = 0.0;
    if (xnext) {
        double v1[1];
        red_get<1>(sc + S_VMV, rs_vmv, v1, sh);
        alpha = rho / v1[0];
    }
    if (type) {
        if (xnext && xsel == (k & 1))
            for (int64_t i = (int64_t)blockIdx.x * VEC_T + threadIdx.x; i < n3; i += stride)
                __builtin_nontemporal_store(__builtin_nontemporal_load(xcur + i) + alpha * __builtin_nontemporal_load(p + i), xnext + i);
        return;
    }
    for (int64_t i = (int64_t)blockIdx.x * VEC_T + threadIdx.x; i < n3; i += stride)
    {
        const double po = PNT ? vld_rmw(p + i) : p[i];
        const double pn = (PNT ? vld_ro(r + i) : r[i]) + beta * po;
        if (PNT) __builtin_nontemporal_store(pn, p + i);
        else p[i] = pn;
        if (xnext) __builtin_nontemporal_store(vld_ro(xcur + i) + alpha * po, xnext + i);
    }
}

struct sr_args {
    int64_t n3, k;
    double *sc;
    int64_t *st;
    double epsf;
    int64_t maxits, its_before_restart;
    int merit_stop;
    int refresh;
    const double *xcur;
    double *xnext;
    double *r, *p, *s;
    const double *w, *bh;
    double *partial;
    fold_args fold;
    red_src rs;
};

__global__ void __launch_bounds__(VEC_T) k_vec_sr(sr_args a) {
    __shared__ double sh[4];
    __shared__ int sh_last;
    const int64_t k = a.k;
    if (a.st[T_ITER_A] < k) return;
    double t3[3];
    red_get<3>(a.sc + S_SR_GAMMA, a.rs, t3, sh);
    const double gamma = t3[0], delta = t3[1], merit = t3[2];
    const double bnorm = a.sc[S_BNORM];
    int type = 0;
    int64_t its = k - 1, xsel = (k - 1) & 1;
    if (!isfinite(gamma)) type = -4;
    else if (k > 1) {
        if (sqrt(gamma) <= a.epsf * bnorm) type = 1;
        else if (k - 1 >= a.maxits && a.maxits > 0) type = 5;
        else if (a.merit_stop && merit >= a.sc[S_PMF0 + ((k - 1) & 1)]) { type = 7; xsel = (k - 2) & 1; }
    }
    double alpha = 0, beta = 0;
    if (!type) {
        const bool restart = k == 1 || ((k - 1) % a.its_before_restart) == 0;
        double pap = delta;
        if (!restart) {
            beta = gamma / a.sc[S_SR_GP0 + ((k - 1) & 1)];
            pap = delta - beta * gamma / a.sc[S_SR_AP0 + ((k - 1) & 1)];
        }
        if (!isfinite(pap) || !isfinite(beta)) type = -4;
        else if (pap <= 0) type = -5;
        else { alpha = gamma / pap; if (!isfinite(alpha)) type = -4; }
        if (type) { its = k; xsel = (k - 1) & 1; }
    }
    if (blockIdx.x == 0 && threadIdx.x == 0) {
        a.sc[S_R2OUT] = gamma;
        if (type) {
            a.st[T_TYPE] = type;
            a.st[T_ITERS] = its;
            a.st[T_XSEL] = xsel;
            a.st[T_ITER_A] = k - 1;
        } else {
            a.sc[S_SR_GP0 + (k & 1)] = gamma;
            a.sc[S_SR_AP0 + (k & 1)] = alpha;
            a.sc[S_PMF0 + (k & 1)] = merit;
        }
    }
    if (type) return;
    double s_mf = 0;
    const int64_t stride = (int64_t)gridDim.x * VEC_T;
    for (int64_t i = (int64_t)blockIdx.x * VEC_T + threadIdx.x; i < a.n3; i += stride) {
        const double ri = a.r[i];
        const double pi = ri + beta * a.p[i];
        const double si = __builtin_nontemporal_load(a.w + i) + beta * a.s[i];
        const double cx = __builtin_nontemporal_load(a.xcur + i) + alpha * pi;
        __builtin_nontemporal_store(pi, a.p + i);
        __builtin_nontemporal_store(si, a.s + i);
        __builtin_nontemporal_store(cx, a.xnext + i);
        if (!a.refresh) {
            const double cr = ri - alpha * si;
            __builtin_nontemporal_store(cr, a.r + i);
            if (a.merit_stop) s_mf -= (cr + a.bh[i]) * cx;
        }
    }
    if (!a.refresh) {
        const double t = block_sum(s_mf, sh);
        if (threadIdx.x == 0) st_agent(a.partial + blockIdx.x, t);
        if (a.fold.counter && fold_arrive(a.fold, &sh_last)) fold_finish<1>(a.fold, a.partial, sh);
    }
}

__global__ void k_result(int64_t n3, int64_t dof0, const int32_t *red, const double *s,
                         const double *x, double *U) {
    const int64_t stride = (int64_t)gridDim.x * blockDim.x;
    for (int64_t i = (int64_t)blockIdx.x * blockDim.x + threadIdx.x; i < n3; i += stride) {
        const int32_t rd = red[dof0 + i];
        if (rd != -1) U[dof0 + i - rd] = s[i] * x[i];
    }
}
__global__ void k_result_full(int64_t n3, const double *s, const double *x, double *full) {
    const int64_t stride = (int64_t)gridDim.x * blockDim.x;
    for (int64_t i = (int64_t)blockIdx.x * blockDim.x + threadIdx.x; i < n3; i += stride)
        full[i] = s[i] * x[i];
}
__global__ void k_compress(int64_t n_dof, const int32_t *red, const double *full, double *U) {
    const int64_t stride = (int64_t)gridDim.x * blockDim.x;
    for (int64_t i = (int64_t)blockIdx.x * blockDim.x + threadIdx.x; i < n_dof; i += stride) {
        const int32_t rd = red[i];
        if (rd != -1) U[i - rd] = full[i];
    }
}
__global__ void k_expand(int64_t n3, int64_t dof0, const int32_t *red, const double *in,
                         const double *div, double *out) {
    const int64_t stride = (int64_t)gridDim.x * blockDim.x;
    for (int64_t i = (int64_t)blockIdx.x * blockDim.x + threadIdx.x; i < n3; i += stride) {
        const int32_t rd = red[dof0 + i];
        double v = rd == -1 ? 0.0 : in[dof0 + i - rd];
        if (div) v /= div[i];
        out[i] = v;
    }
}
__global__ void k_compress_div(int64_t n3, const int32_t *red, const double *s, const double *y,
                               double *out) {
    const int64_t stride = (int64_t)gridDim.x * blockDim.x;
    for (int64_t i = (int64_t)blockIdx.x * blockDim.x + threadIdx.x; i < n3; i += stride) {
        const int32_t rd = red[i];
        if (rd != -1) out[i - rd] = s ? y[i] / s[i] : y[i];
    }
}
__global__ void k_fill(double *p, int64_t n, double v) {
    const int64_t stride = (int64_t)gridDim.x * blockDim.x;
    for (int64_t i = (int64_t)blockIdx.x * blockDim.x + threadIdx.x; i < n; i += stride) p[i] = v;
}
```

### stan_amd/csrc/internal.h

```cpp
#pragma once

#include <hip/hip_runtime.h>
#include <stdint.h>
#include <stdio.h>

#include <atomic>
#include <condition_variable>
#include <functional>
#include <mutex>
#include <string>
#include <unordered_map>
#include <unordered_set>
#include <vector>

#include "../../include/stan_hip.h"

#define STAN_SLICE 64
#define STAN_MAX_INCIDENT 64
#define STAN_MAX_ROW_BLOCKS 96

#define HIPCHK(ctx, call)                                                              \
    do {                                                                               \
        hipError_t e_ = (call);                                                        \
        if (e_ != hipSuccess) {                                                        \
// ... 43 lines not shown
        bytes_avail = 0;
    }
};

struct event_bag {
    std::vector<hipEvent_t> ev;
    hipEvent_t make(unsigned flags = hipEventDefault) {
        hipEvent_t e = nullptr;
        if (hipEventCreateWithFlags(&e, flags) == hipSuccess) ev.push_back(e);
        return e;
    }
    ~event_bag() { for (hipEvent_t e : ev) hipEventDestroy(e); }
};

enum stan_status_slot {
    SS_ERRBITS = 0,
    SS_H_NINC = 1,
    SS_H_NHALO = 2,
    SS_H_NSLOTS = 3,
    SS_H_NBLOCKS = 4,
    SS_H_MAXROW = 5,
    SS_H_COUNT_A = 6,
    SS_H_COUNT_B = 7,
    SS_BAD_ELEM = 8,
    SS_AUX = 9,
    SS_COUNTER = 10,
    SS_H_ERRCOPY = 11,
    SS_MAXDEG = 12,
    SS_NGIANT = 13,
    SS_NBIG = 14,
    SS_WIDTH_SUM = 16,
    SS_WIDTH_MAX = 17,
    SS_H_CG_STATUS = 16,
    SS_H_CG_SCALARS = 40
};

struct stan_cg_ws {
    int64_t ng = 0, n3 = 0;
    double *xb[2] = {nullptr, nullptr}, *p = nullptr, *r = nullptr;
    double *v = nullptr, *w = nullptr, *bh = nullptr, *sv = nullptr;
    double *vw_owner = nullptr;
    static constexpr int NVEC = 8;
    struct slot { double **q; bool gather; };
    slot vec(int i) {
        double **const all[NVEC] = {&xb[0], &xb[1], &p, &r, &v, &w, &bh, &sv};
        return slot{all[i], i < 4};
    }
};

constexpr int STAN_P2P_RING = 4;
constexpr int STAN_P2P_MAXR = 16;
struct stan_p2p_dev {
    int32_t n, me;
    double *mbox[STAN_P2P_MAXR];
    unsigned long long *sig_red[STAN_P2P_MAXR][STAN_P2P_RING];
    unsigned long long *sig_halo[STAN_P2P_MAXR][STAN_P2P_RING];
};
struct stan_p2p {
    int n = 0;
    int wait_mode = 1;
    struct rank_res {
        int device = 0;
        double *mbox = nullptr;
        unsigned long long *sig_red[STAN_P2P_RING] = {}, *sig_halo[STAN_P2P_RING] = {};
        stan_p2p_dev *d_dev = nullptr;
        unsigned long long *d_tick = nullptr;
        int64_t red_calls = 0, halo_calls = 0;
        unsigned long long red_expect[STAN_P2P_RING] = {}, halo_expect[STAN_P2P_RING] = {};
        double *vec[5] = {};
        int64_t nloc = 0;
        std::vector<int> nbr;
        std::vector<int64_t> recv_off;
    };
    std::vector<rank_res> rk;
    bool ipc = false;
    int ipc_me = -1;
    void *ipc_block = nullptr;
    std::vector<void *> ipc_peer_block;
    std::unordered_map<std::string, void *> ipc_open;
    std::unordered_set<std::string> ipc_live;
    std::mutex m;
    std::condition_variable cv;
    int arrived = 0;
    long generation = 0;
    std::atomic<bool> broken{false};
};
int stan_p2p_create(stan_p2p **out, const std::vector<int> &devices, std::string *err);
int stan_p2p_rank_setup(stan_p2p *pp, int rank, std::string *err);
int stan_p2p_rank_finish(stan_p2p *pp, int rank, std::string *err);
void stan_p2p_rank_release(stan_p2p *pp, int rank);
void stan_p2p_destroy(stan_p2p *pp);
void stan_p2p_abort(stan_p2p *pp);
void stan_p2p_dump(stan_p2p *pp, FILE *f);
int stan_p2p_barrier(stan_p2p *pp);
double stan_p2p_stall_seconds();
void stan_p2p_release_own(stan_ctx *ctx);
struct stan_ctx;
int stan_p2p_ipc_setup(stan_ctx *ctx);
void stan_p2p_ipc_release(stan_ctx *ctx);
void stan_p2p_ipc_trim(stan_ctx *ctx);
struct stan_matrix;
int stan_p2p_reduce_slot(stan_ctx *ctx);
int stan_p2p_reduce_wait(stan_ctx *ctx, const unsigned long long **ctr = nullptr, unsigned long long *want = nullptr);
const stan_p2p_dev *stan_p2p_table(stan_ctx *ctx);
const double *stan_p2p_mailbox(stan_ctx *ctx, int slot);
int stan_p2p_publish_vectors(stan_ctx *ctx, const stan_matrix *K, double *const vec[5]);
int stan_p2p_halo_exchange(stan_ctx *ctx, stan_matrix *K, double *d_vec);

struct stan_matrix;
struct stan_group;
struct stan_ctx {
    stan_group *group = nullptr;
    int device = 0;
    hipStream_t stream = nullptr;
    bool own_stream = false;
    std::string err;
    int64_t bad_elem = -1;
    int rank = 0, nranks = 1;
    void *comm = nullptr;
    std::mutex comm_mu;
    std::atomic<bool> comm_broken{false};
    rccl_api nccl;
    stan_p2p *p2p = nullptr;
    bool comm_p2p = false;
    bool result_segment = false;
    bool defer_frees = false;
    bool peers_share_device = false;
    std::vector<void *> deferred;
    bool cg_merit_stop = true;
    int cg_rupdate = 10;
    bool cg_fused_refresh = true;
    bool cg_single_reduce = false;
    int64_t spmv_small_rows = 150000;
    bool cg_defer_x = true;
    bool cols16 = true;
    int vec_store_nt = 3;
    bool cg_fold_reduce = true;
    bool cg_lazy_scaling = true;
    int cg_refine = 1;
    bool overlap_halo = true;
    hipStream_t side = nullptr;
    hipEvent_t ev_a = nullptr, ev_b = nullptr;
    int assembly_mode = 0;
    int row_folding = -1;
    int sell_sigma = 1;
    int placement_tries = 16;
    int64_t placement_max_bytes = 0;
    float prof_placement_ms_best = 0, prof_placement_ms_worst = 0;
    int prof_placement_candidates = 0;
    int prof_placement_moved_vectors = 0;
    int prof_colours = 0;
    int spmv_variant = -1;
    int value_stream_60 = -1;
    bool profiling = false;
    stan_profile prof{};
    double prof_loads_ms[3] = {0, 0, 0};
    double prof_thermal_ms[3] = {0, 0, 0};
    double prof_kg_ms[4] = {0, 0, 0, 0};
    stan_pool pool;
    stan_cg_ws ws;
    std::vector<stan_matrix *> matrices;
    int64_t *h_status = nullptr;
    int64_t *d_status = nullptr;
};
inline bool stan_sharded(const stan_ctx *ctx) { return ctx->comm != nullptr || ctx->nranks > 1; }

constexpr int STAN_NSTREAMS = 4;
struct stan_value_stream {
    int dwords;
    void *padded = nullptr;
    void *folded = nullptr;
    bool refused = false;
};
struct stan_colpack {
    uint32_t *cols16 = nullptr;
    int32_t *colbase = nullptr;
    int32_t *pair_ptr = nullptr;
    uint8_t *packed = nullptr;
    int64_t slots_packed = 0;
    int64_t slots_packed2 = 0;
};

struct stan_matrix {
    stan_ctx *ctx = nullptr;
    std::vector<stan_matrix *> parts;
    int64_t n_dof = 0, n_red = 0;
    int64_t nb_glob = 0;
    int64_t r0 = 0, r1 = 0;
    int64_t u0 = 0, u1 = 0;
    int64_t nloc = 0, nhalo = 0;
    int32_t nslices = 0;
    int64_t nslots = 0;
    int64_t nblocks = 0;
    int32_t max_row_blocks = 0;
    int64_t n_elem_scanned = 0;
    int32_t *d_slot_ptr = nullptr;
    int32_t *d_rowlen = nullptr;
    int32_t *d_rowof = nullptr;
    int32_t *d_posof = nullptr;
    int sigma = 1;
    int32_t *d_cols = nullptr;
    stan_colpack pk;
    stan_value_stream vs[STAN_NSTREAMS] = {{9 * 2}, {9}, {14}, {17}};
    double *vals64() const { return (double *)vs[STAN_PREC_FP64].padded; }
    int32_t *d_fold_ptr = nullptr;
    uint32_t *d_fold_meta = nullptr;
    int4 *d_fold_plan = nullptr;
    int32_t *d_fold_cols = nullptr;
    stan_colpack fold_pk;
    int64_t nfslots = 0;
    bool fold_cols_filled = false;
    int fold_state = 0;
    int32_t *d_red = nullptr;
    uint8_t *d_fixmask = nullptr;
    double *d_scale = nullptr;
    bool scaled = false;
    std::vector<int> nbr;
    std::vector<int64_t> send_off;
    std::vector<int64_t> recv_off;
    int32_t *d_send_rows = nullptr;
    int32_t *d_halo_glob = nullptr;
    double *d_sendbuf = nullptr;
    std::vector<int64_t> row_starts;
    int32_t *d_sl_int = nullptr, *d_sl_bnd = nullptr;
    int32_t n_sl_int = 0, n_sl_bnd = 0;
};

static inline int64_t stan_row_start(int64_t nb, int nranks, int r) {
    if (r >= nranks) return nb;
    const int64_t nsl = (nb + 63) / 64;
    const int64_t s = nsl * r / nranks * 64;
    return s > nb ? nb : s;
}

struct stan_mesh {
    int64_t n_nodes = 0, n_elem = 0, n_dof = 0;
    int32_t n_mat = 0;
    const double *xyz = nullptr, *disp = nullptr;
    const int32_t *node_dof = nullptr;
    const int32_t *conn = nullptr;
    const int32_t *elem_mat = nullptr;
    const uint8_t *elem_type = nullptr;
    const int32_t *red = nullptr;
    const double *mat_E_nu = nullptr;
    stan_mesh chunk(int64_t e0, int64_t e1) const {
        stan_mesh c = *this;
        c.n_elem = e1 - e0; c.conn = conn + 8 * e0; c.elem_mat = elem_mat + e0; c.elem_type = elem_type + e0;
        return c;
    }
};

int stan_scan_exclusive(stan_ctx *ctx, const int32_t *d_in, int64_t *d_out, int64_t n);
int stan_scan_total(stan_ctx *ctx, const int32_t *d_in, int64_t *d_out, int64_t n, int slot);
struct dev_scope;
int stan_compact_collect(stan_ctx *ctx, const int32_t *d_flag, const int64_t *d_rank, int64_t n, int slot, int32_t **out, int64_t *count, dev_scope *tmp = nullptr);
int stan_compact_flags(stan_ctx *ctx, const int32_t *d_flag, int64_t *d_rank, int64_t n, int slot, int32_t **out, int64_t *count, dev_scope *tmp = nullptr);
int stan_slot_ptr_narrow(stan_ctx *ctx, const int64_t *d_ptr64, int64_t n, int32_t **d_ptr32);

int stan_assemble_device(stan_ctx *ctx, const stan_mesh &d, stan_matrix **outK);
int stan_ke_batch_device(stan_ctx *ctx, int64_t n, const double *d_xyz8, double E, double nu,
                         const uint8_t *d_type, double *d_out);

int stan_assemble_colour_scatter(stan_ctx *ctx, stan_matrix *K, int64_t n_elem, const int32_t *d_conn,
                                 const int32_t *d_perm, const double *d_xyz, const int32_t *d_elem_mat,
                                 const uint8_t *d_elem_type, const double *d_lamG, const int64_t *d_ptr,
                                 const int32_t *d_list, long long *d_bad);

int stan_cg_device(stan_ctx *ctx, stan_matrix *K, const double *d_F, double eps_f,
                   int32_t max_its, int32_t precision_mode, double *d_U, int32_t *term,
                   int32_t *iters, double *rel_res);
int stan_cg_multi_device(stan_ctx *ctx, stan_matrix *K, int32_t n_rhs, const double *d_F, double eps_f, int32_t max_its,
                         int32_t precision_mode, double *d_U, int32_t *term, int32_t *iters, double *rel_res);
int stan_spmv_reduced(stan_ctx *ctx, stan_matrix *K, const double *d_x, double *d_y);
int stan_matrix_diagonal(stan_ctx *ctx, stan_matrix *K, double *d_diag);
int stan_spmv_bench_device(stan_ctx *ctx, stan_matrix *K, int32_t precision_mode, int32_t reps,
                           double *avg_ms);
int stan_stream_bench_device(stan_ctx *ctx, stan_matrix *K, int32_t reps, double *avg_ms, int64_t *bytes);
int stan_spmv_local(stan_ctx *ctx, stan_matrix *K, const double *d_x, double *d_y);
int stan_matrix_make_fp32(stan_ctx *ctx, stan_matrix *K);
int stan_matrix_make_folded(stan_ctx *ctx, stan_matrix *K, int32_t stream_kind, bool plan_only = false);
void stan_matrix_drop_folded_values(stan_ctx *ctx, stan_matrix *K);
void stan_matrix_abandon_folding(stan_ctx *ctx, stan_matrix *K);
int stan_matrix_make_fx48(stan_ctx *ctx, stan_matrix *K);
int stan_matrix_alloc_stream(stan_ctx *ctx, stan_matrix *K, int32_t kind, int64_t slots, void **out, bool folded = false, bool second_copy = false);
int stan_matrix_alloc_s60(stan_ctx *ctx, stan_matrix *K, uint32_t **out);
int stan_stream_encode(stan_ctx *ctx, int32_t kind, int64_t nslots, const double *d_vals, uint32_t *d_out, int64_t *refused);
int stan_matrix_encode_s60(stan_ctx *ctx, stan_matrix *K, uint32_t *blk);
int stan_stream60_roundtrip_device(stan_ctx *ctx, int64_t n, const double *in, double *out, int64_t *refused);
int stan_matrix_make_cols16(stan_ctx *ctx, stan_matrix *K);
int stan_pack_columns(stan_ctx *ctx, int32_t nslices, int64_t nslots, const int32_t *d_slot_ptr, const int32_t *d_cols, stan_colpack *out,
                      int64_t nloc = 0, const int32_t *d_rowof = nullptr, const int32_t *d_rowlen = nullptr);
int stan_matrix_ensure_scaled(stan_ctx *ctx, stan_matrix *K);
inline int64_t gather_len(const stan_matrix *K) {
    const int64_t npad = (int64_t)K->nslices * 64;
    return 3 * (npad > K->nloc + K->nhalo ? npad : K->nloc + K->nhalo);
}
int stan_cg_workspace(stan_ctx *ctx, const stan_matrix *K);
void stan_cg_workspace_free(stan_ctx *ctx);
int stan_cg_workspace_move(stan_ctx *ctx, const stan_matrix *K, bool commit, stan_cg_ws *saved);
size_t stan_cg_products_bytes(const stan_ctx *ctx);
void stan_cg_products_set(stan_ctx *ctx, double *block, double *saved[3]);
void stan_cg_products_adopt(stan_ctx *ctx, double *block, size_t bytes, double *saved[3]);

int stan_recover_device(stan_ctx *ctx, const stan_mesh &d, double *d_strain, double *d_stress, double *d_elem_forces = nullptr,
                        double *d_R = nullptr);

// ... 225 lines not shown
```

### stan_amd/csrc/spmv_kernels.inc

```

template <bool NT, typename T>
__device__ __forceinline__ T ld_stream(const T *p) {
    if constexpr (NT) return __builtin_nontemporal_load(p);
    else return *p;
}

struct s60_t { uint32_t w; };
template <typename VT> struct vstream { static constexpr int STRIDE = 9 * 64; static constexpr bool FX = false, P60 = false; };
template <> struct vstream<uint32_t> { static constexpr int STRIDE = 14 * 64; static constexpr bool FX = true, P60 = false; };
template <> struct vstream<s60_t> { static constexpr int STRIDE = S60_ROWS * 64; static constexpr bool FX = false, P60 = true; };

template <bool NT, typename VT>
__device__ __forceinline__ void load9(const VT *vp, double a[9]) {
    if constexpr (vstream<VT>::FX) {
        uint32_t lo[9], hw[5];
#pragma unroll
        for (int j = 0; j < 9; j++) lo[j] = ld_stream<NT>(vp + j * 64);
#pragma unroll
        for (int m = 0; m < 5; m++) hw[m] = ld_stream<NT>(vp + (9 + m) * 64);
#pragma unroll
        for (int j = 0; j < 9; j++) {
            const uint32_t h = (j & 1) ? (hw[j >> 1] >> 16) : (hw[j >> 1] & 0xffffu);
            a[j] = __hiloint2double((int)(0x43300000u | h), (int)lo[j]) - FX48_BIAS;
        }
// ... 195 lines not shown
        if (DOT) dot_terms<DOT>(x, row, y0, y1, y2, d, e);
    }
    if (DOT) dot_reduce<DOT>(d, e, partial, poff, fold, sh, &sh_last);
}

__global__ void __launch_bounds__(256)
k_value_stream(int32_t nslices, const int32_t *__restrict__ slot_ptr, const double *__restrict__ vals, double *sink) {
    __shared__ double sh[4];
    const int lane = threadIdx.x & 63;
    const int64_t slice = xcd_chunked<32>(blockIdx.x) * 4 + (threadIdx.x >> 6);
    double s0 = 0, s1 = 0, s2 = 0;
    if (slice < nslices) {
        const int32_t k0 = slot_ptr[slice], k1 = slot_ptr[slice + 1];
        const double *vp = vals + (int64_t)k0 * vstream<double>::STRIDE + lane;
        int32_t k = k0;
        for (; k + 1 < k1; k += 2) {
            double a[9], b[9];
            load9<true, double>(vp, a);
            load9<true, double>(vp + vstream<double>::STRIDE, b);
            s0 += a[0] + a[1] + a[2] + b[0] + b[1] + b[2];
            s1 += a[3] + a[4] + a[5] + b[3] + b[4] + b[5];
            s2 += a[6] + a[7] + a[8] + b[6] + b[7] + b[8];
            vp += 2 * vstream<double>::STRIDE;
        }
        if (k < k1) {
            double a[9];
            load9<true, double>(vp, a);
            s0 += a[0] + a[1] + a[2]; s1 += a[3] + a[4] + a[5]; s2 += a[6] + a[7] + a[8];
        }
    }
    const double t = block_sum(s0 + s1 + s2, sh);
    if (threadIdx.x == 0) sink[blockIdx.x] = t;
}

template <int DOT>
__global__ void __launch_bounds__(256)
k_spmv_first(int32_t nslices, int64_t nloc, const int32_t *__restrict__ slot_ptr, const int32_t *__restrict__ rowof,
             const int32_t *__restrict__ cols, double *__restrict__ vals, const double *__restrict__ s,
             const double *__restrict__ x, double *__restrict__ y, double *partial,
             const int64_t *st, int64_t kiter, fold_args fold, colstream cs) {
    __shared__ double sh[4];
    __shared__ int sh_last;
    (void)st; (void)kiter;
    const int lane = threadIdx.x & 63;
    const int64_t slice = xcd_chunked<32>(blockIdx.x) * 4 + (threadIdx.x >> 6);
    double y0 = 0, y1 = 0, y2 = 0;
    const int64_t row = row_at(slice, nslices, rowof, lane, nloc);
    if (slice < nslices) {
        const int32_t k0 = slot_ptr[slice], k1 = slot_ptr[slice + 1];
        const double sr0 = s[3 * row], sr1 = s[3 * row + 1], sr2 = s[3 * row + 2];
#define STAN_SPMV_FIRST_BLOCK(C, VP)                                                                   \
    {                                                                                                  \
        double a[9];                                                                                   \
        load9<true, double>(VP, a);                                                                    \
        const double sc0_ = s[3 * (C)], sc1_ = s[3 * (C) + 1], sc2_ = s[3 * (C) + 2];                  \
        a[0] *= sr0 * sc0_; a[1] *= sr0 * sc1_; a[2] *= sr0 * sc2_;                                    \
        a[3] *= sr1 * sc0_; a[4] *= sr1 * sc1_; a[5] *= sr1 * sc2_;                                    \
        a[6] *= sr2 * sc0_; a[7] *= sr2 * sc1_; a[8] *= sr2 * sc2_;                                    \
        _Pragma("unroll") for (int j = 0; j < 9; j++) __builtin_nontemporal_store(a[j], (VP) + j * 64); \
        const double x0 = x[3 * (C)], x1 = x[3 * (C) + 1], x2 = x[3 * (C) + 2];                        \
        y0 += a[0] * x0 + a[1] * x1 + a[2] * x2;                                                       \
        y1 += a[3] * x0 + a[4] * x1 + a[5] * x2;                                                       \
        y2 += a[6] * x0 + a[7] * x1 + a[8] * x2;                                                       \
    }
        walk_slots<true, 1, 9 * 64>(cs, cols, slice, lane, k0, k0, k1, vals,
                                    [&](int64_t c, double *vp) { STAN_SPMV_FIRST_BLOCK(c, vp) });
#undef STAN_SPMV_FIRST_BLOCK
        if (row < nloc) store_row<true>(y, row, y0, y1, y2);
    }
    if (DOT) {
        double d = 0, e = 0;
        if (slice < nslices && row < nloc) dot_terms<DOT>(x, row, y0, y1, y2, d, e);
        dot_reduce<DOT>(d, e, partial, 0, fold, sh, &sh_last);
    }
}

template <typename VT, int DOT>
__global__ void __launch_bounds__(256)
k_spmv_small(int32_t nslices, int64_t nloc, const int32_t *__restrict__ slot_ptr, const int32_t *__restrict__ rowof,
             const int32_t *__restrict__ cols, const VT *__restrict__ vals,
             const double *__restrict__ x, double *__restrict__ y, double *partial,
             const int64_t *st, int64_t kiter, const int32_t *__restrict__ slist, int32_t nlist,
             int32_t poff, fold_args fold, colstream cs) {
    __shared__ double sh[4];
    __shared__ int sh_last;
    __shared__ double acc[3][4][64];
    if (stopped(st, kiter)) { fold_skip(fold); return; }
    constexpr bool NT = false;
    const int lane = threadIdx.x & 63, w = threadIdx.x >> 6;
    const int64_t slice = slice_at(blockIdx.x, slist, nlist, nslices);
    double y0 = 0, y1 = 0, y2 = 0;
    const int64_t row = row_at(slice, nslices, rowof, lane, nloc);
    if (slice < nslices) {
        const int32_t k0 = slot_ptr[slice], k1 = slot_ptr[slice + 1];
        const int pmode = cs.packed ? (int)cs.ok[slice] : 0;
        const bool packed = pmode != 0;
        const bool cb = pmode == 2 && ((cs.cmask[slice] >> lane) & 1ull);
        const int64_t pp = packed ? (int64_t)cs.pair_ptr[slice] : 0;
        for (int32_t k = k0 + w; k < k1; k += 4) {
            int64_t c;
            if (packed) {
                const uint32_t wd = cs.packed[(pp + ((k - k0) >> 1)) * 64 + lane];
                const int32_t b0 = cs.base[k], q0 = cs.base2[k];
                c = (int64_t)(cb ? q0 : b0) + (int64_t)(((k - k0) & 1) ? (wd >> 16) : (wd & 0xffffu));
            } else
                c = cols[(int64_t)k * 64 + lane];
            const VT *vp = vals + (int64_t)k * vstream<VT>::STRIDE + lane;
            STAN_SPMV_BLOCK(c, vp)
        }
    }
    acc[0][w][lane] = y0; acc[1][w][lane] = y1; acc[2][w][lane] = y2;
    __syncthreads();
    double d = 0, e = 0;
    if (w == 0) {
        y0 = ((acc[0][0][lane] + acc[0][1][lane]) + acc[0][2][lane]) + acc[0][3][lane];
        y1 = ((acc[1][0][lane] + acc[1][1][lane]) + acc[1][2][lane]) + acc[1][3][lane];
        y2 = ((acc[2][0][lane] + acc[2][1][lane]) + acc[2][2][lane]) + acc[2][3][lane];
        if (slice < nslices && row < nloc) {
            store_row<NT>(y, row, y0, y1, y2);
            if (DOT) dot_terms<DOT>(x, row, y0, y1, y2, d, e);
        }
    }
    if (DOT) dot_reduce<DOT>(d, e, partial, poff, fold, sh, &sh_last);
}

template <typename VT>
__global__ void __launch_bounds__(256) __attribute__((amdgpu_waves_per_eu(1, 4)))
k_spmv2(int32_t nslices, int64_t nloc, const int32_t *__restrict__ slot_ptr, const int32_t *__restrict__ rowof,
        const int32_t *__restrict__ cols, const VT *__restrict__ vals,
        const double *__restrict__ x, const double *__restrict__ x2, double *__restrict__ y,
        double *__restrict__ y2, double *partial, const int64_t *st, int64_t kiter,
        const int32_t *__restrict__ slist, int32_t nlist, int32_t poff, fold_args fold, colstream cs) {
    __shared__ double sh[4];
    __shared__ int sh_last;
    if (stopped(st, kiter)) { fold_skip(fold); return; }
    const int lane = threadIdx.x & 63;
    int64_t bid = blockIdx.x;
    bid = xcd_chunked<32>(bid);
    const int64_t slice = slice_at(bid * 4 + (threadIdx.x >> 6), slist, nlist, nslices);
    double y0 = 0, y1 = 0, yy2 = 0, z0 = 0, z1 = 0, z2 = 0;
    const int64_t row = row_at(slice, nslices, rowof, lane, nloc);
    if (slice < nslices) {
        const int32_t k0 = slot_ptr[slice], k1 = slot_ptr[slice + 1];
#define STAN_SPMV2_BLOCK(C, VP)                                                       \
    {                                                                                 \
        double a[9];                                                                  \
        load9<true, VT>(VP, a);                                                       \
        double x0 = x[3 * (C)], x1 = x[3 * (C) + 1], xx2 = x[3 * (C) + 2];            \
        double u0 = x2[3 * (C)], u1 = x2[3 * (C) + 1], u2 = x2[3 * (C) + 2];          \
        if (vstream<VT>::FX) {                                                        \
            x0 *= FX48_INV; x1 *= FX48_INV; xx2 *= FX48_INV;                          \
            u0 *= FX48_INV; u1 *= FX48_INV; u2 *= FX48_INV;                           \
        }                                                                             \
        y0 += a[0] * x0 + a[1] * x1 + a[2] * xx2;                                     \
        y1 += a[3] * x0 + a[4] * x1 + a[5] * xx2;                                     \
        yy2 += a[6] * x0 + a[7] * x1 + a[8] * xx2;                                    \
        z0 += a[0] * u0 + a[1] * u1 + a[2] * u2;                                      \
        z1 += a[3] * u0 + a[4] * u1 + a[5] * u2;                                      \
        z2 += a[6] * u0 + a[7] * u1 + a[8] * u2;                                      \
    }
        walk_slots<true, 2, vstream<VT>::STRIDE>(cs, cols, slice, lane, k0, k0, k1, vals,
                                                 [&](int64_t c, const VT *vp) { STAN_SPMV2_BLOCK(c, vp) });
#undef STAN_SPMV2_BLOCK
        if (row < nloc) {
            store_row<true>(y, row, y0, y1, yy2);
            store_row<true>(y2, row, z0, z1, z2);
        }
    }
    double d = 0, e = 0;
    if (slice < nslices && row < nloc) dot_terms<1>(x, row, y0, y1, yy2, d, e);
    dot_reduce<1>(d, e, partial, poff, fold, sh, &sh_last);
}


template <typename VT, int DOT, int NRHS>
__global__ void __launch_bounds__(256) __attribute__((amdgpu_waves_per_eu(1, (NRHS == 2 ? 4 : 5))))
k_spmv_fold(int32_t nslices, int64_t nloc, const int32_t *__restrict__ fold_ptr, const int32_t *__restrict__ rowof,
            const uint32_t *__restrict__ meta, const int32_t *__restrict__ cols, const VT *__restrict__ vals,
            const double *__restrict__ x, const double *__restrict__ x2, double *__restrict__ y, double *__restrict__ y2,
            double *partial, const int64_t *st, int64_t kiter, const int32_t *__restrict__ slist, int32_t nlist,
            int32_t poff, fold_args fold, colstream cs) {
    __shared__ double sh[4];
    __shared__ int sh_last;
    __shared__ double fsh[4][3 * NRHS][64];
    if (stopped(st, kiter)) { fold_skip(fold); return; }
    const int lane = threadIdx.x & 63, w = threadIdx.x >> 6;
    int64_t bid = blockIdx.x;
    bid = xcd_chunked<32>(bid);
    const int64_t slice = slice_at(bid * 4 + w, slist, nlist, nslices);
    double y0 = 0, y1 = 0, yy2 = 0, z0 = 0, z1 = 0, z2 = 0;
    double f0 = 0, f1 = 0, f2 = 0, g0 = 0, g1 = 0, g2 = 0;
    const int64_t row = row_at(slice, nslices, rowof, lane, nloc);
    uint32_t m = 0;
    if (slice < nslices) {
        m = meta[slice * 64 + lane];
        const int32_t own = (int32_t)(m & 0xffffu);
        const int32_t k0 = fold_ptr[slice], k1 = fold_ptr[slice + 1];
        const int32_t *cp = cols + (int64_t)k0 * 64 + lane;
        const VT *vp = vals + (int64_t)k0 * vstream<VT>::STRIDE + lane;
#define STAN_FOLD_LOAD(S, C, VP)                                                                \
        double a##S[9];                                                                         \
        load9<true, VT>(VP, a##S);                                                              \
        double x0##S = x[3 * (C)], x1##S = x[3 * (C) + 1], x2##S = x[3 * (C) + 2];              \
        double u0##S = 0, u1##S = 0, u2##S = 0;                                                 \
        if (NRHS == 2) { u0##S = x2[3 * (C)]; u1##S = x2[3 * (C) + 1]; u2##S = x2[3 * (C) + 2]; }
#define STAN_FOLD_MATH(S, KL)                                                                   \
    {                                                                                           \
        if (vstream<VT>::FX) { x0##S *= FX48_INV; x1##S *= FX48_INV; x2##S *= FX48_INV; }       \
        const double t0 = a##S[0] * x0##S + a##S[1] * x1##S + a##S[2] * x2##S;                  \
        const double t1 = a##S[3] * x0##S + a##S[4] * x1##S + a##S[5] * x2##S;                  \
        const double t2 = a##S[6] * x0##S + a##S[7] * x1##S + a##S[8] * x2##S;                  \
        const bool mine = (KL) < own;                                                           \
        y0 += mine ? t0 : 0.0; y1 += mine ? t1 : 0.0; yy2 += mine ? t2 : 0.0;                   \
        f0 += mine ? 0.0 : t0; f1 += mine ? 0.0 : t1; f2 += mine ? 0.0 : t2;                    \
        if (NRHS == 2) {                                                                        \
            if (vstream<VT>::FX) { u0##S *= FX48_INV; u1##S *= FX48_INV; u2##S *= FX48_INV; }   \
            const double s0 = a##S[0] * u0##S + a##S[1] * u1##S + a##S[2] * u2##S;              \
            const double s1 = a##S[3] * u0##S + a##S[4] * u1##S + a##S[5] * u2##S;              \
            const double s2 = a##S[6] * u0##S + a##S[7] * u1##S + a##S[8] * u2##S;              \
            z0 += mine ? s0 : 0.0; z1 += mine ? s1 : 0.0; z2 += mine ? s2 : 0.0;                \
            g0 += mine ? 0.0 : s0; g1 += mine ? 0.0 : s1; g2 += mine ? 0.0 : s2;                \
        }                                                                                       \
    }
        if (cs.packed && cs.ok[slice] == 1) {
            const uint32_t *cq = cs.packed + (int64_t)cs.pair_ptr[slice] * 64 + lane;
            const int32_t *bp = cs.base + __builtin_amdgcn_readfirstlane(k0);
            int32_t k = k0;
            uint32_t wd = __builtin_nontemporal_load(cq);
            for (; k + 1 < k1; k += 2) {
                const uint32_t wn = __builtin_nontemporal_load(k + 2 < k1 ? cq + 64 : cq);
                const int64_t c = (int64_t)bp[0] + (int64_t)(wd & 0xffffu);
                const int64_t c2 = (int64_t)bp[1] + (int64_t)(wd >> 16);
                STAN_FOLD_LOAD(A, c, vp)
                STAN_FOLD_LOAD(B, c2, vp + vstream<VT>::STRIDE)
                STAN_FOLD_MATH(A, k - k0)
                STAN_FOLD_MATH(B, k - k0 + 1)
                cq += 64;
                bp += 2;
                vp += 2 * vstream<VT>::STRIDE;
                wd = wn;
            }
            if (k < k1) {
                const int64_t c = (int64_t)bp[0] + (int64_t)(wd & 0xffffu);
                STAN_FOLD_LOAD(A, c, vp)
                STAN_FOLD_MATH(A, k - k0)
            }
        } else {
            int32_t k = k0;
            for (; k + 1 < k1; k += 2) {
                const int64_t c = __builtin_nontemporal_load(cp), c2 = __builtin_nontemporal_load(cp + 64);
                STAN_FOLD_LOAD(A, c, vp)
                STAN_FOLD_LOAD(B, c2, vp + vstream<VT>::STRIDE)
                STAN_FOLD_MATH(A, k - k0)
                STAN_FOLD_MATH(B, k - k0 + 1)
                cp += 128;
                vp += 2 * vstream<VT>::STRIDE;
            }
            if (k < k1) {
                const int64_t c = __builtin_nontemporal_load(cp);
                STAN_FOLD_LOAD(A, c, vp)
                STAN_FOLD_MATH(A, k - k0)
            }
        }
#undef STAN_FOLD_LOAD
#undef STAN_FOLD_MATH
    }
    const int nh = (int)(m >> 24);
    if (__any(nh > 0)) {
        fsh[w][0][lane] = f0; fsh[w][1][lane] = f1; fsh[w][2][lane] = f2;
        if (NRHS == 2) { fsh[w][3][lane] = g0; fsh[w][4][lane] = g1; fsh[w][5][lane] = g2; }
        __builtin_amdgcn_fence(__ATOMIC_RELEASE, "wavefront");
        __builtin_amdgcn_wave_barrier();
        __builtin_amdgcn_fence(__ATOMIC_ACQUIRE, "wavefront");
        const int hfirst = (int)((m >> 16) & 0xffu);
        for (int h = 0; h < nh; h++) {
            const int j = hfirst - h;
            y0 += fsh[w][0][j]; y1 += fsh[w][1][j]; yy2 += fsh[w][2][j];
            if (NRHS == 2) { z0 += fsh[w][3][j]; z1 += fsh[w][4][j]; z2 += fsh[w][5][j]; }
        }
    }
    if (slice < nslices && row < nloc) {
        store_row<true>(y, row, y0, y1, yy2);
        if (NRHS == 2) store_row<true>(y2, row, z0, z1, z2);
    }
    if (DOT) {
        double d = 0, e = 0;
        if (slice < nslices && row < nloc) dot_terms<DOT>(x, row, y0, y1, yy2, d, e);
        dot_reduce<DOT>(d, e, partial, poff, fold, sh, &sh_last);
    }
}
```

### stan_amd/hip.py

```python
import ctypes as C
import os

import numpy as np

_HERE = os.path.dirname(os.path.abspath(__file__))
LIB_PATH = os.environ.get("STAN_HIP_LIB") or os.path.join(_HERE, "lib", "libstan_hip.so")

HEX8_G1, HEX8_G2 = 1, 2
N_SCALARS = 24
PREC_FP64, PREC_MIXED, PREC_FIXED48 = 0, 1, 2
OPT_CG_MERIT_STOP, OPT_CG_RUPDATE, OPT_SPMV_VARIANT, OPT_OVERLAP_HALO, OPT_ASSEMBLY_MODE = 1, 2, 3, 4, 5
OPT_CG_FUSED_REFRESH = 6
OPT_POOL = 7
OPT_PLACEMENT_TRIES = 8
OPT_POOL_MAX_BYTES = 9
OPT_CG_SINGLE_REDUCE = 10
OPT_CG_FOLD_REDUCE = 11
OPT_VEC_STORE_NT = 12
OPT_PACKED_COLUMNS = 13
OPT_CG_DEFER_X = 14
OPT_SPMV_SMALL = 15
OPT_PLACEMENT_MAX_BYTES = 16
OPT_SELL_SIGMA = 17
OPT_COMM_P2P = 18
OPT_ROW_FOLDING = 19
OPT_CG_REFINE = 20
OPT_CG_LAZY_SCALING = 21
OPT_VALUE_STREAM_60 = 22
VALUE_STREAM_60 = 3
E_HIP, E_ARG, E_ALLOC, E_DETJ, E_DOF_LAYOUT, E_VALENCE, E_COMM, E_UNSUPPORTED = (
    -1, -2, -3, -4, -5, -6, -7, -8)

EXPORTS = [
    "stan_hip_init", "stan_hip_init_multi", "stan_hip_destroy", "stan_hip_last_error", "stan_hip_last_bad_element",
    "stan_hip_set_stream", "stan_hip_comm_unique_id", "stan_hip_comm_init",
    "stan_hip_assemble_hex8", "stan_hip_assemble_hex8_dev", "stan_hip_matrix_free",
    "stan_hip_cg_solve", "stan_hip_cg_solve_dev", "stan_hip_cg_solve_multi", "stan_hip_cg_solve_multi_dev", "stan_hip_matrix_info", "stan_hip_ke_hex8",
    "stan_hip_ke_hex8_batch", "stan_hip_matrix_to_csr", "stan_hip_spmv", "stan_hip_spmv_bench", "stan_hip_stream_bench",
    "stan_hip_stream60_roundtrip",
    "stan_hip_set_profiling", "stan_hip_get_profile", "stan_hip_set_option", "stan_hip_recover_hex8", "stan_hip_recover_hex8_dev",
    "stan_hip_nodal_forces_hex8", "stan_hip_pool_info",
    "stan_hip_matrix_plan", "stan_hip_spmv_local", "stan_hip_comm_info", "stan_hip_comm_library",
    "stan_hip_matrix_part_info", "stan_hip_get_profile_rank", "stan_hip_device_info", "stan_hip_matrix_diagonal",
    "stan_hip_recover_hex8_keep", "stan_hip_results_map", "stan_hip_results_free",
    "stan_hip_result_scalars_hex8", "stan_hip_results_scalars",
    "stan_hip_internal_forces_hex8", "stan_hip_internal_forces_hex8_dev",
    "stan_hip_load_vector_hex8", "stan_hip_load_vector_hex8_dev", "stan_hip_load_vector_times",
    "stan_hip_thermal_load_hex8", "stan_hip_thermal_load_hex8_dev", "stan_hip_thermal_load_times",
    "stan_hip_thermal_stress_hex8", "stan_hip_thermal_stress_hex8_dev", "stan_hip_results_thermal_stress",
    "stan_hip_lumped_mass_hex8", "stan_hip_lumped_mass_hex8_dev", "stan_hip_modes", "stan_hip_modes_dev",
    "stan_hip_block_gram", "stan_hip_block_rotate",
    "stan_hip_matrix_shifted", "stan_hip_matrix_shifted_dev", "stan_hip_transient", "stan_hip_transient_dev",
    "stan_hip_newmark_predict", "stan_hip_newmark_correct",
    "stan_hip_kg_hex8_batch", "stan_hip_geometric_stiffness_hex8", "stan_hip_geometric_stiffness_hex8_dev",
    "stan_hip_geometric_stiffness_times", "stan_hip_buckling", "stan_hip_buckling_dev", "stan_hip_buckling_rotate",
]
LAB_EXPORTS = ["stan_hip_csr_spmv_bench", "stan_hip_lab_placement_map", "stan_hip_lab_placement_variants", "stan_hip_lab_placement_alloc", "stan_hip_lab_placement_rounds", "stan_hip_lab_placement_cross", "stan_hip_lab_incg_penalty", "stan_hip_lab_placement_vecalloc", "stan_hip_lab_placement_vecshape", "stan_hip_lab_pairing_pmc"]


class MatrixInfo(C.Structure):
    _fields_ = [("n_dof", C.c_int64), ("n_reduced", C.c_int64), ("n_block_rows", C.c_int64),
                ("row_begin", C.c_int64), ("row_end", C.c_int64), ("n_halo", C.c_int64),
                ("n_blocks", C.c_int64), ("n_slots", C.c_int64), ("bytes_matrix", C.c_int64),
                ("scaled", C.c_int32), ("max_row_blocks", C.c_int32), ("n_elements_on_device", C.c_int64),
                ("sell_sigma", C.c_int32), ("folded_slots_permille", C.c_int32)]


class Profile(C.Structure):
    _fields_ = [("assemble_ms", C.c_double), ("symbolic_ms", C.c_double),
                ("numeric_ms", C.c_double), ("cg_ms", C.c_double), ("spmv_ms_total", C.c_double),
                ("spmv_launches", C.c_int64), ("spmv_bytes", C.c_int64),
                ("cg_iteration_vector_bytes", C.c_int64), ("iterations", C.c_int32),
                ("termination_type", C.c_int32), ("assembly_colours", C.c_int32),
                ("value_stream", C.c_int32), ("spmv2_ms_total", C.c_double), ("spmv2_launches", C.c_int64),
                ("loop_kernel_launches", C.c_int64), ("loop_collectives", C.c_int64),
                ("loop_iterations_enqueued", C.c_int64), ("placement_candidates", C.c_int32),
                ("placement_ms_best", C.c_float), ("placement_ms_worst", C.c_float),
                ("col_slots_packed", C.c_int64), ("placement_moved_vectors", C.c_int32), ("repacked_streams", C.c_int32),
                ("loop_stream_waits", C.c_int64), ("comm_reduce_ms_total", C.c_double),
                ("comm_reduce_calls", C.c_int64), ("comm_halo_ms_total", C.c_double), ("comm_halo_calls", C.c_int64),
                ("rel_residual_recurrence", C.c_double), ("rel_residual_fp64", C.c_double), ("refine_passes", C.c_int32),
                ("fp64_products", C.c_int32), ("fp64_products_ms", C.c_double),
                ("scalars_cell_ms", C.c_double), ("scalars_list_ms", C.c_double), ("scalars_point_ms", C.c_double),
                ("forces_elem_ms", C.c_double), ("forces_list_ms", C.c_double), ("forces_gather_ms", C.c_double)]


class _Sums(C.Structure):

    def as_dict(self):
        return {k: (list(getattr(self, k)) if k.endswith("_sum") else getattr(self, k)) for k, _ in self._fields_}


class Equilibrium(_Sums):
    _fields_ = [("reaction_sum", C.c_double * 3), ("load_sum", C.c_double * 3), ("fint_sum", C.c_double * 3),
                ("residual_norm2", C.c_double), ("load_norm2", C.c_double), ("residual_max", C.c_double),
                ("residual_max_dof", C.c_int64), ("n_fixed", C.c_int64)]


class LoadSums(_Sums):
    _fields_ = [("load_sum", C.c_double * 3), ("free_sum", C.c_double * 3), ("volume", C.c_double), ("area", C.c_double),
                ("n_fixed", C.c_int64), ("n_faces", C.c_int64)]


class ThermalSums(_Sums):
    _fields_ = [("load_sum", C.c_double * 3), ("free_sum", C.c_double * 3), ("volume", C.c_double), ("dT_integral", C.c_double),
                ("n_fixed", C.c_int64)]


class MassSums(_Sums):
    _fields_ = [("total_mass", C.c_double), ("volume", C.c_double), ("free_sum", C.c_double * 3), ("fixed_sum", C.c_double * 3),
                ("n_fixed", C.c_int64)]


class ModesReport(C.Structure):
    _fields_ = [("block", C.c_int32), ("outer", C.c_int32), ("converged", C.c_int32), ("cg_worst_type", C.c_int32),
                ("cg_iterations", C.c_int64), ("max_rho", C.c_double), ("solve_ms", C.c_double), ("product_ms", C.c_double),
                ("block_ms", C.c_double), ("gram_ms", C.c_double), ("rotate_ms", C.c_double)]

    def as_dict(self):
        return {k: getattr(self, k) for k, _ in self._fields_}


class BucklingReport(C.Structure):
    _fields_ = [("block", C.c_int32), ("outer", C.c_int32), ("converged", C.c_int32), ("n_positive", C.c_int32),
                ("cg_worst_type", C.c_int32), ("reserved", C.c_int32), ("cg_iterations", C.c_int64),
                ("lowest_negative_factor", C.c_double), ("max_rho", C.c_double), ("solve_ms", C.c_double),
                ("product_ms", C.c_double), ("block_ms", C.c_double), ("gram_ms", C.c_double), ("rotate_ms", C.c_double)]

    def as_dict(self):
        return {k: getattr(self, k) for k, _ in self._fields_}


class TransientReport(C.Structure):
    _fields_ = [("steps", C.c_int32), ("failed_step", C.c_int32), ("cg_worst_type", C.c_int32), ("cg_min_iterations", C.c_int32),
                ("cg_max_iterations", C.c_int32), ("reserved", C.c_int32), ("cg_iterations", C.c_int64), ("sigma", C.c_double),
                ("shift_ms", C.c_double), ("solve_ms", C.c_double), ("product_ms", C.c_double), ("step_ms", C.c_double),
                ("predict_ms", C.c_double), ("correct_ms", C.c_double)]

    def as_dict(self):
        return {k: getattr(self, k) for k, _ in self._fields_}


def newmark_coef(dt, beta_N=0.25, gamma=0.5, alpha_R=0.0, beta_R=0.0):
    return np.array([1.0 / (beta_N * dt * dt), gamma / (beta_N * dt), 1.0 / (beta_N * dt), 1.0 / (2.0 * beta_N) - 1.0,
                     gamma / beta_N - 1.0, dt * (gamma / (2.0 * beta_N) - 1.0), alpha_R, beta_R])


class StanHipError(RuntimeError):
    def __init__(self, code, msg):
        super().__init__("libstan_hip error %d: %s" % (code, msg))
        self.code = code


_lib = None


def load():
    global _lib
    if _lib is None:
        if not os.path.exists(LIB_PATH):
            raise RuntimeError(
                "%s is missing: run `python -c 'import __graft_entry__ as g; g.build()'` "
                "(there is no CPU fallback)" % LIB_PATH)
        try:
            import torch
        except ImportError:
            pass
        _lib = C.CDLL(LIB_PATH)
        _lib.stan_hip_last_error.restype = C.c_char_p
        _lib.stan_hip_last_bad_element.restype = C.c_int64
        _lib.stan_hip_destroy.restype = None
        _lib.stan_hip_matrix_free.restype = None
    return _lib


def _ptr(a, t):
    if a is None:
        return None
    return a.ctypes.data_as(C.POINTER(t))


def _dev(p, t):
    return C.cast(C.c_void_p(int(p)), C.POINTER(t))


def _opt(p, t=C.c_double):
    return None if p is None else _dev(p, t)


_MESH = dict(xyz=np.float64, disp=np.float64, node_dof=np.int32, conn=np.int32, elem_mat=np.int32, elem_type=np.uint8,
             mat_E_nu=np.float64, red=np.int32)


def _mesh(**arrays):
    out = {k: np.ascontiguousarray(a, dtype=_MESH[k]) for k, a in arrays.items()}
    return [a.reshape(-1, 8 if k == "conn" else 2) if k in ("conn", "mat_E_nu") else a for k, a in out.items()]


class Context:
    def __init__(self, device=0, devices=None):
        self.lib = load()
        h = C.c_void_p()
        if devices is not None:
            arr = (C.c_int * len(devices))(*devices)
            rc = self.lib.stan_hip_init_multi(C.c_int(len(devices)), arr, C.byref(h))
        else:
            rc = self.lib.stan_hip_init(C.c_int(device), C.byref(h))
        if rc != 0:
            self.lib.stan_hip_last_error.argtypes = [C.c_void_p]
            msg = self.lib.stan_hip_last_error(None)
            raise StanHipError(rc, msg.decode() if msg else "stan_hip_init failed")
        self.h = h
        self.lib.stan_hip_last_error.argtypes = [C.c_void_p]
        self.lib.stan_hip_last_bad_element.argtypes = [C.c_void_p]
        self.device = device

    def close(self):
        if getattr(self, "h", None):
            self.lib.stan_hip_destroy(self.h)
            self.h = None

    def __del__(self):
        try:
            self.close()
        except Exception:
            pass

    def _chk(self, rc):
        if rc != 0:
            raise StanHipError(rc, self.lib.stan_hip_last_error(self.h).decode())

    def last_bad_element(self):
        return int(self.lib.stan_hip_last_bad_element(self.h))

    def set_stream(self, stream_ptr):
        self._chk(self.lib.stan_hip_set_stream(self.h, C.c_void_p(stream_ptr)))

    def set_option(self, option, value):
        self._chk(self.lib.stan_hip_set_option(self.h, C.c_int32(option), C.c_int64(value)))

    def set_profiling(self, on=True):
        self._chk(self.lib.stan_hip_set_profiling(self.h, C.c_int32(1 if on else 0)))

    def stream60_roundtrip(self, values):
        values = np.ascontiguousarray(values, dtype=np.float64)
        out, refused = np.zeros_like(values), C.c_int64(0)
        self._chk(self.lib.stan_hip_stream60_roundtrip(self.h, C.c_int64(values.size), _ptr(values, C.c_double),
                                                       _ptr(out, C.c_double), C.byref(refused)))
        return out, refused.value

    def profile(self):
        p = Profile()
        self._chk(self.lib.stan_hip_get_profile(self.h, C.byref(p)))
        return {k: getattr(p, k) for k, _ in Profile._fields_}

    def profile_rank(self, rank):
        p = Profile()
        self._chk(self.lib.stan_hip_get_profile_rank(self.h, C.c_int32(rank), C.byref(p)))
        return {k: getattr(p, k) for k, _ in Profile._fields_}

    def device_info(self, rank=0):
        o, b = C.c_int32(-1), C.create_string_buffer(32)
        self._chk(self.lib.stan_hip_device_info(self.h, C.c_int32(rank), C.byref(o), b))
        return o.value, b.value.decode()

    def pool_info(self):
        b, n = C.c_int64(0), C.c_int64(0)
        self._chk(self.lib.stan_hip_pool_info(self.h, C.byref(b), C.byref(n)))
        return b.value, n.value

    def unique_id(self):
        buf = C.create_string_buffer(128)
        rc = self.lib.stan_hip_comm_unique_id(buf)
        if rc != 0:
            raise StanHipError(rc, "ncclGetUniqueId failed")
        return bytes(buf.raw)

    def comm_init(self, rank, nranks, uid):
        if uid is None:
            self._chk(self.lib.stan_hip_comm_init(self.h, C.c_int(rank), C.c_int(nranks), None))
            return
        buf = C.create_string_buffer(bytes(uid), 128)
        self._chk(self.lib.stan_hip_comm_init(self.h, C.c_int(rank), C.c_int(nranks), buf))

    def comm_info(self):
        v, n, r, p = C.c_int32(0), C.c_int32(0), C.c_int32(0), C.c_int32(0)
        self._chk(self.lib.stan_hip_comm_info(self.h, C.byref(v), C.byref(n), C.byref(r), C.byref(p)))
        buf, reused = C.create_string_buffer(4096), C.c_int32(0)
        self._chk(self.lib.stan_hip_comm_library(self.h, buf, C.c_int64(4096), C.byref(reused)))
        return dict(rccl_version=v.value, comm_ranks=n.value, comm_rank=r.value, p2p=bool(p.value),
                    library=buf.value.decode(), library_reused=bool(reused.value))

    def ke_hex8(self, xyz8, E, nu, etype):
        xyz8 = np.ascontiguousarray(xyz8, dtype=np.float64).reshape(24)
        out = np.zeros(576)
        self._chk(self.lib.stan_hip_ke_hex8(self.h, _ptr(xyz8, C.c_double), C.c_double(E),
                                            C.c_double(nu), C.c_int32(etype),
                                            _ptr(out, C.c_double)))
        return out.reshape(24, 24)

    def ke_hex8_batch(self, xyz8, E, nu, etypes):
        xyz8 = np.ascontiguousarray(xyz8, dtype=np.float64).reshape(-1, 24)
        n = xyz8.shape[0]
        etypes = np.ascontiguousarray(etypes, dtype=np.uint8)
        out = np.zeros((n, 576))
        self._chk(self.lib.stan_hip_ke_hex8_batch(self.h, C.c_int64(n), _ptr(xyz8, C.c_double),
                                                  C.c_double(E), C.c_double(nu),
                                                  _ptr(etypes, C.c_uint8), _ptr(out, C.c_double)))
        return out.reshape(n, 24, 24)

    def kg_hex8_batch(self, xyz8, u8, E, nu, etypes):
        xyz8 = np.ascontiguousarray(xyz8, dtype=np.float64).reshape(-1, 24)
        u8 = np.ascontiguousarray(u8, dtype=np.float64).reshape(-1, 24)
        n = xyz8.shape[0]
        etypes = np.ascontiguousarray(etypes, dtype=np.uint8).reshape(-1)
        if u8.shape[0] != n or etypes.shape[0] != n:
            raise ValueError("kg_hex8_batch: xyz8, u8 must be [n, 24] and etypes [n]")
        out = np.zeros((n, 36))
        self._chk(self.lib.stan_hip_kg_hex8_batch(self.h, C.c_int64(n), _ptr(xyz8, C.c_double), _ptr(u8, C.c_double),
                                                  C.c_double(E), C.c_double(nu), _ptr(etypes, C.c_uint8), _ptr(out, C.c_double)))
        return out

    def geometric_stiffness_times(self):
        ms = (C.c_double * 4)()
        self._chk(self.lib.stan_hip_geometric_stiffness_times(self.h, ms))
        return dict(kg_elem_ms=ms[0], kg_layout_ms=ms[1], kg_list_ms=ms[2], kg_gather_ms=ms[3])

    def buckling(self, K, G, n_modes, tol=0.0, max_outer=0, solve_eps=0.0, solve_max_its=0):
        N = K.info()["n_reduced"]
        k = max(int(n_modes), 1)
        fac, phi, rho, rep = np.zeros(k), np.zeros((k, N)), np.zeros(k), BucklingReport()
        self._chk(self.lib.stan_hip_buckling(
            self.h, K.k, G.k, C.c_int32(int(n_modes)), C.c_double(tol), C.c_int32(max_outer), C.c_double(solve_eps),
            C.c_int32(solve_max_its), _ptr(fac, C.c_double), _ptr(phi, C.c_double), _ptr(rho, C.c_double), C.byref(rep)))
        return fac, phi, rho, rep.as_dict()

    def buckling_dev(self, K, G, n_modes, d_factor, d_phi, d_rho, tol=0.0, max_outer=0, solve_eps=0.0, solve_max_its=0):
        rep = BucklingReport()
        self._chk(self.lib.stan_hip_buckling_dev(
            self.h, K.k, G.k, C.c_int32(int(n_modes)), C.c_double(tol), C.c_int32(max_outer), C.c_double(solve_eps),
            C.c_int32(solve_max_its), _opt(d_factor), _opt(d_phi), _opt(d_rho), C.byref(rep)))
        return rep.as_dict()

    def buckling_rotate(self, Z, W, Y, D, Q, mu):
        Z, W, Y, Q = (np.ascontiguousarray(x, dtype=np.float64) for x in (Z, W, Y, Q))
        D = np.ascontiguousarray(D, dtype=np.float64).reshape(-1)
        mu = np.ascontiguousarray(mu, dtype=np.float64).reshape(-1)
        if Z.ndim != 2 or W.shape != Z.shape or Y.shape != Z.shape or D.shape[0] != Z.shape[1] or Q.shape != (Z.shape[0],) * 2 or mu.shape[0] != Z.shape[0]:
            raise ValueError("buckling_rotate: Z, W, Y must be [q, N], D [N], Q [q, q], mu [q]")
        q, N = Z.shape
        X, KX, R, r2, kx2 = np.zeros((q, N)), np.zeros((q, N)), np.zeros((q, N)), np.zeros(q), np.zeros(q)
        self._chk(self.lib.stan_hip_buckling_rotate(
            self.h, C.c_int64(N), C.c_int32(q), _ptr(Z, C.c_double), _ptr(W, C.c_double), _ptr(Y, C.c_double), _ptr(D, C.c_double),
            _ptr(Q, C.c_double), _ptr(mu, C.c_double), _ptr(X, C.c_double), _ptr(KX, C.c_double), _ptr(R, C.c_double),
            _ptr(r2, C.c_double), _ptr(kx2, C.c_double)))
        return X, KX, R, r2, kx2

    def recover_hex8(self, xyz, disp, conn, elem_mat, elem_type, mat_E_nu):
        xyz, disp, conn, elem_mat, elem_type, mat_E_nu = _mesh(
            xyz=xyz, disp=disp, conn=conn, elem_mat=elem_mat, elem_type=elem_type, mat_E_nu=mat_E_nu)
        ne = conn.shape[0]
        strain = np.zeros((ne, 8, 6))
        stress = np.zeros((ne, 8, 6))
        self._chk(self.lib.stan_hip_recover_hex8(
            self.h, C.c_int64(xyz.shape[0]), _ptr(xyz, C.c_double), _ptr(disp, C.c_double),
            C.c_int64(ne), _ptr(conn, C.c_int32), _ptr(elem_mat, C.c_int32),
            _ptr(elem_type, C.c_uint8), C.c_int32(mat_E_nu.shape[0]), _ptr(mat_E_nu, C.c_double),
            _ptr(strain, C.c_double), _ptr(stress, C.c_double)))
        return strain, stress

    def recover_hex8_dev(self, n_nodes, d_xyz, d_disp, n_elem, d_conn, d_elem_mat, d_elem_type, mat_E_nu, d_strain, d_stress):
        mat_E_nu = np.ascontiguousarray(mat_E_nu, dtype=np.float64).reshape(-1, 2)
        self._chk(self.lib.stan_hip_recover_hex8_dev(
            self.h, C.c_int64(n_nodes), _dev(d_xyz, C.c_double), _dev(d_disp, C.c_double), C.c_int64(n_elem),
            _dev(d_conn, C.c_int32), _dev(d_elem_mat, C.c_int32), _dev(d_elem_type, C.c_uint8),
            C.c_int32(mat_E_nu.shape[0]), _ptr(mat_E_nu, C.c_double), _dev(d_strain, C.c_double), _dev(d_stress, C.c_double)))

    def recover_hex8_keep(self, xyz, disp, conn, elem_mat, elem_type, mat_E_nu):
        xyz, disp, conn, elem_mat, elem_type, mat_E_nu = _mesh(
            xyz=xyz, disp=disp, conn=conn, elem_mat=elem_mat, elem_type=elem_type, mat_E_nu=mat_E_nu)
        h = C.c_void_p()
        self._chk(self.lib.stan_hip_recover_hex8_keep(
            self.h, C.c_int64(xyz.shape[0]), _ptr(xyz, C.c_double), _ptr(disp, C.c_double),
            C.c_int64(conn.shape[0]), _ptr(conn, C.c_int32), _ptr(elem_mat, C.c_int32),
            _ptr(elem_type, C.c_uint8), C.c_int32(mat_E_nu.shape[0]), _ptr(mat_E_nu, C.c_double), C.byref(h)))
        return Results(self, h, conn.shape[0])

    def _scalars(self, call, disp, conn, sel, point, cell):
        disp = np.ascontiguousarray(disp, dtype=np.float64).reshape(-1, 3)
        conn = np.ascontiguousarray(conn, dtype=np.int32).reshape(-1, 8)
        sel = np.ascontiguousarray(range(N_SCALARS) if sel is None else sel, dtype=np.int32).reshape(-1)
        nn, ne, ns = disp.shape[0], conn.shape[0], sel.shape[0]
        pt = np.zeros((ns, nn)) if point else None
        ce = np.zeros((ns, 3, ne)) if cell else None
        self._chk(call(C.c_int64(nn), _ptr(disp, C.c_double), C.c_int64(ne), _ptr(conn, C.c_int32), C.c_int32(ns),
                       _ptr(sel, C.c_int32), _ptr(pt, C.c_double), _ptr(ce, C.c_double)))
        return pt, ce

    def result_scalars(self, disp, conn, strain, stress, sel=None, point=True, cell=True):
        strain = np.ascontiguousarray(strain, dtype=np.float64)
        stress = np.ascontiguousarray(stress, dtype=np.float64)
        ne = np.asarray(conn).size // 8
        if strain.size != ne * 48 or stress.size != ne * 48:
            raise ValueError("result_scalars: strain / stress must be [n_elem, 8, 6]")
        return self._scalars(
            lambda nn, d, n_e, c, ns, s, pt, ce: self.lib.stan_hip_result_scalars_hex8(
                self.h, nn, d, n_e, c, _ptr(strain, C.c_double), _ptr(stress, C.c_double), ns, s, pt, ce),
            disp, conn, sel, point, cell)

    def nodal_forces_hex8(self, xyz, disp, node_dof, conn, elem_mat, elem_type, mat_E_nu):
        xyz, disp, node_dof, conn, elem_mat, elem_type, mat_E_nu = _mesh(
            xyz=xyz, disp=disp, node_dof=node_dof, conn=conn, elem_mat=elem_mat, elem_type=elem_type, mat_E_nu=mat_E_nu)
        ne, n_dof = conn.shape[0], xyz.shape[0] * 3
        f = np.zeros((ne, 24))
        R = np.zeros(n_dof)
        self._chk(self.lib.stan_hip_nodal_forces_hex8(
            self.h, C.c_int64(xyz.shape[0]), _ptr(xyz, C.c_double), _ptr(disp, C.c_double),
            _ptr(node_dof, C.c_int32), C.c_int64(ne), _ptr(conn, C.c_int32), _ptr(elem_mat, C.c_int32),
            _ptr(elem_type, C.c_uint8), C.c_int32(mat_E_nu.shape[0]), _ptr(mat_E_nu, C.c_double),
            C.c_int64(n_dof), _ptr(f, C.c_double), _ptr(R, C.c_double)))
        return f, R

# ... 571 lines not shown
```

Before: 6.697 million.

## Defer CG solution updates via a ring of search directions and stream60 refresh SpMV

Adds an x-ring mode for CG. Each iteration's search direction p and its alpha are kept in a ring of W+1 buffers, and x is updated in batched flushes that sum several alpha*p terms in one pass. This replaces the per-iteration x read/write, cutting vector traffic per iteration at the cost of extra memory and flush kernels. It also lets the fused refresh SpMV (two-vector product) use the compressed 60-bit value stream through a new k_spmv2 path with s60_row accumulation. Both modes are enabled automatically for large matrices.

Result: faster. 6.794 million (median of 6 runs) (+1.5%).

```diff
diff --git a/include/stan_hip.h b/include/stan_hip.h
--- a/include/stan_hip.h
+++ b/include/stan_hip.h
@@ -56,9 +56,13 @@
 #define STAN_OPT_POOL 7
 #define STAN_OPT_POOL_MAX_BYTES 9
 #define STAN_OPT_VALUE_STREAM_60 22
+#define STAN_OPT_CG_X_RING 23
+#define STAN_OPT_CG_REFRESH_60 24
 #define STAN_OPT_SPMV_VARIANT 3
 int stan_hip_set_option(stan_ctx *ctx, int32_t option, int64_t value);
 int stan_hip_pool_info(stan_ctx *ctx, int64_t *bytes_parked, int64_t *blocks_parked);
+
+int stan_hip_cg_loop_info(stan_ctx *ctx, int32_t *x_ring_window, int64_t *x_ring_flushes, int32_t *refresh_stream);
 
 int stan_hip_comm_unique_id(char id[128]);
 int stan_hip_comm_init(stan_ctx *ctx, int rank, int nranks, const char id[128]);
diff --git a/stan_amd/csrc/api.hip b/stan_amd/csrc/api.hip
--- a/stan_amd/csrc/api.hip
+++ b/stan_amd/csrc/api.hip
@@ -130,6 +130,8 @@
         }
     }
     else if (option == STAN_OPT_VALUE_STREAM_60 && value >= -1 && value <= 1) ctx->value_stream_60 = (int)value;
+    else if (option == STAN_OPT_CG_X_RING && value >= -1 && value <= 1) ctx->cg_x_ring = (int)value;
+    else if (option == STAN_OPT_CG_REFRESH_60 && value >= -1 && value <= 1) ctx->cg_refresh_60 = (int)value;
     else if (option == STAN_OPT_OVERLAP_HALO) ctx->overlap_halo = value != 0;
     else if (option == STAN_OPT_SELL_SIGMA && value >= 1 && value <= 32) ctx->sell_sigma = (int)value;
     else if (option == STAN_OPT_PLACEMENT_TRIES && value >= 1 && value <= 64) ctx->placement_tries = (int)value;
@@ -146,6 +148,15 @@
     if (ctx->group) ctx = stan_group_rank0(ctx);
     if (bytes_parked) *bytes_parked = (int64_t)ctx->pool.bytes_avail;
     if (blocks_parked) *blocks_parked = (int64_t)ctx->pool.avail.size();
+    return STAN_OK;
+}
+
+int stan_hip_cg_loop_info(stan_ctx *ctx, int32_t *x_ring_window, int64_t *x_ring_flushes, int32_t *refresh_stream) {
+    if (!ctx) return STAN_E_ARG;
+    if (ctx->group) ctx = stan_group_rank0(ctx);
+    if (x_ring_window) *x_ring_window = ctx->prof_x_ring_window;
+    if (x_ring_flushes) *x_ring_flushes = ctx->prof_x_ring_flushes;
+    if (refresh_stream) *refresh_stream = ctx->prof_refresh_stream;
     return STAN_OK;
 }
 
diff --git a/stan_amd/csrc/cg.hip b/stan_amd/csrc/cg.hip
--- a/stan_amd/csrc/cg.hip
+++ b/stan_amd/csrc/cg.hip
@@ -6,6 +6,7 @@
 
 #include "internal.h"
 #include "s60.h"
+#include "x_ring.h"
 #include "p2p_device.h"
 #include "fx48.h"
 
@@ -166,6 +167,11 @@
     const colstream cs = colstream_of(ctx, K->pk, K->nslots);
     if (s60) {
         const s60_t *vals = (const s60_t *)(a.vals ? a.vals : K->vs[a.kind].padded);
+        if (a.x2) {
+            hipLaunchKernelGGL((k_spmv2<s60_t>), dim3(grid), dim3(256), 0, stream, K->nslices, K->nloc, K->d_slot_ptr, K->d_rowof, K->d_cols,
+                               vals, a.x, a.x2, a.y, a.y2, a.partial, a.st, a.k, slist, nlist, poff, fold, cs);
+            return grid;
+        }
         auto launch = [&](auto var) {
             hipLaunchKernelGGL((k_spmv<s60_t, 1, decltype(var)::value>), dim3(grid), dim3(256), 0, stream, K->nslices, K->nloc, K->d_slot_ptr,
                                K->d_rowof, K->d_cols, vals, a.x, a.y, a.partial, a.st, a.k, slist, nlist, poff, fold, cs);
@@ -316,6 +322,12 @@
     bool reduced = false;
     uint32_t *pend60 = nullptr;
     int64_t n60 = 0;
+    bool refresh60 = false;
+    int refresh_stream = -1;
+    int ring_w = 0;
+    double *ring = nullptr, *ring_alpha = nullptr;
+    int64_t ring_flushed = 0, n_flush = 0;
+    double *ring_slot(int64_t j) const { return ring + (int64_t)xring_slot(j, ring_w) * ng; }
     ~cg_run() { if (pend60) stan_dfree(ctx, pend60); }
     int refine = 0;
     int64_t n3 = 0, npad = 0, ng = 0, dof0 = 0;
@@ -386,8 +398,9 @@
             if (!K->vs[STAN_VALUE_STREAM_60].padded) plan.stream60_unavailable();
             STANCHK(rc);
         }
-        const bool s60 = plan.stream60 && !pend60 && !x2 && dot == 1 && !extra && !lazy_scale && kind == STAN_PREC_FP64;
-        if (s60) { kind = STAN_VALUE_STREAM_60; n60++; }
+        const bool s60 = plan.stream60 && !pend60 && (!x2 || refresh60) && dot == 1 && !extra && !lazy_scale && kind == STAN_PREC_FP64;
+        if (s60) { kind = STAN_VALUE_STREAM_60; if (!x2) n60++; }
+        if (x2) refresh_stream = kind;
         span.begin(st_, k);
         auto go = [&](int which, hipStream_t s, bool last) -> unsigned {
             n_launch++;
@@ -425,6 +438,8 @@
     }
 
     int setup();
+    int setup_x_ring();
+    void flush_x_ring(int64_t k, int64_t last_enqueued);
     int begin_pass(bool from_F, double eps_pass, bool *done);
     int iterate(double eps_pass, int32_t max_its_pass);
     int pass(bool from_F, double eps_pass, int32_t max_its_pass);
@@ -466,6 +481,7 @@
         STANCHK(folded_copy(STAN_PREC_FP64, true));
         plan.fold_planned(K);
     }
+    refresh60 = ctx->cg_refresh_60 > 0 || (ctx->cg_refresh_60 < 0 && K->nb_glob > STREAM60_AUTO_ROWS);
     lazy_scale = plan.may_lazy_scale;
     if (lazy_scale) STANCHK(ensure_scale_vector(ctx, K));
     else STANCHK(ensure_scaled(ctx, K));
@@ -506,6 +522,7 @@
     p2p_tab = p2p ? stan_p2p_table(ctx) : nullptr;
     vg = vec_grid(n3);
     its_before_restart = K->n_red > 0 ? K->n_red : 1;
+    STANCHK(setup_x_ring());
     split = dist && ctx->overlap_halo && K->d_sl_bnd != nullptr;
     if (split && !ctx->side) {
         HIPCHK(ctx, hipStreamCreateWithFlags(&ctx->side, hipStreamNonBlocking));
@@ -518,12 +535,50 @@
     return STAN_OK;
 }
 
+int cg_run::setup_x_ring() {
+    ring_w = 0;
+    ctx->prof_x_ring_window = 0;
+    ctx->prof_x_ring_flushes = 0;
+    const bool applies = precision_mode == STAN_PREC_FP64 && !dist && !sr && ctx->cg_defer_x && !ctx->cg_merit_stop &&
+                         ctx->cg_fused_refresh && ctx->cg_rupdate != 1 && n3 > 0;
+    if (!applies || ctx->cg_x_ring == 0 || (ctx->cg_x_ring < 0 && K->nb_glob <= STREAM60_AUTO_ROWS)) return STAN_OK;
+    const int W = xring_window(ctx->cg_rupdate);
+    const size_t bytes = (size_t)(W + 1) * (size_t)ng * 8;
+    const stan_pool &pool = ctx->pool;
+    bool room = false;
+    if (pool.enabled && bytes >= stan_pool::MIN_BYTES)
+        for (const stan_pool::blk &b : pool.avail) room = room || (b.cap >= bytes && b.cap <= bytes + bytes / 2);
+    if (!room) {
+        size_t free_b = 0, total_b = 0;
+        if (hipMemGetInfo(&free_b, &total_b) != hipSuccess) { (void)hipGetLastError(); return STAN_OK; }
+        room = free_b >= bytes + (bytes > total_b / 16 ? bytes : total_b / 16);
+    }
+    if (!room) return STAN_OK;
+    void *blk = nullptr;
+    if (stan_dmalloc_bytes(ctx, &blk, bytes, false) != STAN_OK) { ctx->err.clear(); return STAN_OK; }
+    bufs.p.push_back(blk);
+    ring = (double *)blk;
+    STANCHK(bufs.alloc(&ring_alpha, (size_t)(W + 1)));
+    ring_w = W;
+    for (int s = 0; s <= W && ng > n3; s++) HIPCHK(ctx, hipMemsetAsync(ring + (int64_t)s * ng + n3, 0, (size_t)(ng - n3) * 8, st_));
+    return STAN_OK;
+}
+void cg_run::flush_x_ring(int64_t k, int64_t last_enqueued) {
+    xring_args a;
+    a.n3 = n3; a.ng = ng; a.k = k;
+    a.first = ring_flushed + 1; a.last = k - 1; a.last_enqueued = last_enqueued;
+    a.W = ring_w; a.ring = ring; a.alpha = ring_alpha; a.x = xb[0]; a.st = stt;
+    hipLaunchKernelGGL(k_xring_flush, dim3(vg), dim3(VEC_T), 0, st_, a);
+    n_launch++; n_flush++;
+    if (k > 0) ring_flushed = k - 1;
+}
+
 int cg_run::begin_pass(bool from_F, double eps_pass, bool *done) {
     {
         const fold_args f = vec_fold(sc + S_VMV, p2p_to(0, true));
         if (from_F)
             hipLaunchKernelGGL(k_init, dim3(vg), dim3(VEC_T), 0, st_, n3, dof0, K->d_red, d_F, K->d_scale,
-                               bh, xb[0], r, p, partial, f);
+                               bh, xb[0], r, ring_w ? ring_slot(1) : p, partial, f);
         else
             hipLaunchKernelGGL(k_init_b, dim3(vg), dim3(VEC_T), 0, st_, n3, (const double *)r, bh, xb[0], r, p, partial, f);
         reduce_if_unfolded((int)vg, 1, sc + S_VMV, p2p_to(0, true));
@@ -555,6 +610,10 @@
         if (rc == STAN_OK) rc = exchange_sums(sc + S_SR_GAMMA, 3, &rs_sr);
     }
     const int chunk = dist ? CHUNK_DIST : CHUNK;
+    if (ring_w) {
+        ring_flushed = 0;
+        HIPCHK(ctx, hipMemsetAsync(stt + T_FLUSHED, 0, 8, st_));
+    }
     while (!done && rc == STAN_OK) {
         for (int c = 0; c < chunk && k < chunk_poll::hard_cap; c++, k++) {
             const bool refresh = rupdate > 0 && (k % rupdate) == 0;
@@ -585,7 +644,10 @@
                 continue;
             }
             const bool fused = refresh && ctx->cg_fused_refresh && !refresh64;
-            rc = product(p, fused ? xb[(k - 1) & 1] : nullptr, v, 1, sc + S_VMV, k, p2p_to(0, true), plan.vs);
+            double *const pk = ring_w ? ring_slot(k) : p;
+            double *const xprev = ring_w ? xb[0] : xb[(k - 1) & 1];
+            if (ring_w && xring_flush_due(k, ring_flushed, ring_w, refresh)) flush_x_ring(k, 0);
+            rc = product(pk, fused ? xprev : nullptr, v, 1, sc + S_VMV, k, p2p_to(0, true), plan.vs);
             if (rc) break;
             rc = exchange_sums(sc + S_VMV, 1, &rs_vmv);
             if (rc) break;
@@ -594,7 +656,7 @@
             a.rs_vmv = rs_vmv;
             a.n3 = n3; a.k = k; a.sc = sc; a.st = stt;
             a.xcur = xb[(k - 1) & 1]; a.xnext = xb[k & 1];
-            a.r = r; a.p = p; a.v = v; a.w = w; a.bh = bh; a.partial = partial;
+            a.r = r; a.p = pk; a.v = v; a.w = w; a.bh = bh; a.partial = partial;
             a.refresh = refresh ? (fused ? 2 : 1) : 0;
             a.merit = ctx->cg_merit_stop ? 1 : 0;
             a.defer_x = (ctx->cg_defer_x && !a.merit && a.refresh != 1) ? 1 : 0;
@@ -613,8 +675,14 @@
             if (rc) break;
             const double *ux = a.defer_x ? a.xcur : nullptr;
             double *uxn = a.defer_x ? a.xnext : nullptr;
-            hipLaunchKernelGGL((ctx->vec_store_nt & 1) ? k_update<true> : k_update<false>, dim3(vg), dim3(VEC_T), 0, st_, n3, k, sc, stt,
-                               eps_pass, (int64_t)max_its_pass, its_before_restart, ctx->cg_merit_stop ? 1 : 0, r, p, ux, uxn, rs_r2, rs_vmv);
+            if (ring_w)
+                hipLaunchKernelGGL(((ctx->vec_store_nt & 1) ? k_update<true, true> : k_update<false, true>), dim3(vg), dim3(VEC_T), 0, st_, n3, k, sc, stt,
+                                   eps_pass, (int64_t)max_its_pass, its_before_restart, 0, r, pk, (const double *)nullptr, (double *)nullptr,
+                                   rs_r2, rs_vmv, ring_slot(k + 1), ring_alpha + xring_slot(k, ring_w));
+            else
+                hipLaunchKernelGGL(((ctx->vec_store_nt & 1) ? k_update<true, false> : k_update<false, false>), dim3(vg), dim3(VEC_T), 0, st_, n3, k, sc, stt,
+                                   eps_pass, (int64_t)max_its_pass, its_before_restart, ctx->cg_merit_stop ? 1 : 0, r, p, ux, uxn, rs_r2, rs_vmv,
+                                   (double *)nullptr, (double *)nullptr);
             n_launch++;
         }
         if (rc) break;
@@ -633,13 +701,14 @@
     hipError_t e = hipStreamSynchronize(st_);
     if (rc) return rc;
     if (e != hipSuccess) { ctx->err = std::string("cg: ") + hipGetErrorString(e); return STAN_E_HIP; }
+    if (ring_w) flush_x_ring(0, k - 1);
     HIPCHK(ctx, hipMemcpyAsync(h_st, stt, T_NSTAT * 8, hipMemcpyDeviceToHost, st_));
     HIPCHK(ctx, hipMemcpyAsync(h_sc, sc, S_NSCAL * 8, hipMemcpyDeviceToHost, st_));
     HIPCHK(ctx, hipStreamSynchronize(st_));
     pass_type = (int)h_st[T_TYPE];
     pass_its = h_st[T_ITERS];
     if (pass_type == 0) { pass_type = 5; pass_its = k - 1; h_st[T_XSEL] = (k - 1) & 1; }
-    xfin = xb[h_st[T_XSEL] & 1];
+    xfin = ring_w ? xb[0] : xb[h_st[T_XSEL] & 1];
     return STAN_OK;
 }
 
@@ -700,6 +769,9 @@
     if (ctx->profiling) hipEventRecord(ev1, st_);
     HIPCHK(ctx, hipStreamSynchronize(st_));
 
+    ctx->prof_x_ring_window = ring_w;
+    ctx->prof_x_ring_flushes = n_flush;
+    ctx->prof_refresh_stream = refresh_stream;
     if (term_out) *term_out = type;
     if (iters_out) *iters_out = (int32_t)(its > chunk_poll::hard_cap ? chunk_poll::hard_cap : its);
     if (rel_res_out) *rel_res_out = rel64 >= 0 ? rel64 : rel_rec;
@@ -729,6 +801,7 @@
     pf.col_slots_packed = ctx->cols16 && K->pk.cols16 ? K->pk.slots_packed : 0;
     pf.value_stream = stream;
     pf.cg_iteration_vector_bytes = 3 * K->nloc * 8 * ((ctx->cg_defer_x && !ctx->cg_merit_stop ? 8 : 9) + (ctx->cg_merit_stop ? 1 : 0));
+    if (ring_w) pf.cg_iteration_vector_bytes = 3 * K->nloc * 8 * (7 * (int64_t)ring_w + 2) / ring_w;
     pf.loop_kernel_launches = n_launch;
     pf.loop_collectives = n_coll;
     pf.loop_stream_waits = n_wait;
diff --git a/stan_amd/csrc/cg_reduce_device.inc b/stan_amd/csrc/cg_reduce_device.inc
--- a/stan_amd/csrc/cg_reduce_device.inc
+++ b/stan_amd/csrc/cg_reduce_device.inc
@@ -9,7 +9,9 @@
        S_SR_GAMMA = 9, S_SR_DELTA = 10, S_SR_MERIT = 11, S_SR_GP0 = 12, S_SR_GP1 = 13, S_SR_AP0 = 14,
        S_SR_AP1 = 15,
        S_CHK_R2 = 16, S_CHK_MF = 17, S_NSCAL = 24 };
-enum { T_ITER_A = 0, T_ITER_B = 1, T_TYPE = 2, T_ITERS = 3, T_XSEL = 4, T_NSTAT = 8 };
+enum { T_ITER_A = 0, T_ITER_B = 1, T_TYPE = 2, T_ITERS = 3, T_XSEL = 4,
+       T_FLUSHED = 5,
+       T_NSTAT = 8 };
 
 __device__ __forceinline__ double wave_sum(double v) {
 #pragma unroll
diff --git a/stan_amd/csrc/cg_vector_kernels.inc b/stan_amd/csrc/cg_vector_kernels.inc
--- a/stan_amd/csrc/cg_vector_kernels.inc
+++ b/stan_amd/csrc/cg_vector_kernels.inc
@@ -109,12 +109,12 @@
     if (fold.counter && fold_arrive(fold, &sh_last)) fold_finish<2>(fold, partial, sh);
 }
 
-template <bool PNT>
+template <bool PNT, bool RING>
 __global__ void __launch_bounds__(VEC_T)
 k_update(int64_t n3, int64_t k, double *sc, int64_t *st, double epsf, int64_t maxits,
          int64_t its_before_restart, int merit_stop, const double *r, double *p,
          const double *xcur, double *xnext ,
-         red_src rs_r2, red_src rs_vmv) {
+         red_src rs_r2, red_src rs_vmv, double *pnext, double *alpha_out) {
     __shared__ double sh[4];
     if (st[T_ITER_A] < k || st[T_ITER_B] <= k) return;
     double t2[2];
@@ -147,10 +147,21 @@
     }
     const int64_t stride = (int64_t)gridDim.x * VEC_T;
     double alpha = 0.0;
-    if (xnext) {
+    if (RING || xnext) {
         double v1[1];
         red_get<1>(sc + S_VMV, rs_vmv, v1, sh);
         alpha = rho / v1[0];
+    }
+    if constexpr (RING) {
+        if (blockIdx.x == 0 && threadIdx.x == 0) *alpha_out = alpha;
+        if (type) return;
+        for (int64_t i = (int64_t)blockIdx.x * VEC_T + threadIdx.x; i < n3; i += stride) {
+            const double po = PNT ? vld_rmw(p + i) : p[i];
+            const double pn = (PNT ? vld_ro(r + i) : r[i]) + beta * po;
+            if (PNT) __builtin_nontemporal_store(pn, pnext + i);
+            else pnext[i] = pn;
+        }
+        return;
     }
     if (type) {
         if (xnext && xsel == (k & 1))
@@ -166,6 +177,57 @@
         else p[i] = pn;
         if (xnext) __builtin_nontemporal_store(vld_ro(xcur + i) + alpha * po, xnext + i);
     }
+}
+
+struct xring_args {
+    int64_t n3, ng;
+    int64_t k;
+    int64_t first, last;
+    int64_t last_enqueued;
+    int W;
+    const double *ring;
+    const double *alpha;
+    double *x;
+    int64_t *st;
+};
+template <int N>
+__device__ __forceinline__ void xring_sum(const xring_args &a, int64_t first) {
+    const double *q[N];
+    double al[N];
+#pragma unroll
+    for (int m = 0; m < N; m++) {
+        const int s = xring_slot(first + m, a.W);
+        q[m] = a.ring + (int64_t)s * a.ng;
+        al[m] = a.alpha[s];
+    }
+    const int64_t stride = (int64_t)gridDim.x * VEC_T;
+    for (int64_t i = (int64_t)blockIdx.x * VEC_T + threadIdx.x; i < a.n3; i += stride) {
+        double pv[N];
+#pragma unroll
+        for (int m = 0; m < N; m++) pv[m] = __builtin_nontemporal_load(q[m] + i);
+        double x = __builtin_nontemporal_load(a.x + i);
+#pragma unroll
+        for (int m = 0; m < N; m++) x = __builtin_fma(al[m], pv[m], x);
+        __builtin_nontemporal_store(x, a.x + i);
+    }
+}
+__global__ void __launch_bounds__(VEC_T) k_xring_flush(xring_args a) {
+    int64_t first = a.first, last = a.last;
+    if (a.k > 0) {
+        if (stopped(a.st, a.k)) return;
+    } else {
+        first = a.st[T_FLUSHED] + 1;
+        last = xring_final_iterate(a.st[T_TYPE], a.st[T_ITERS], a.st[T_XSEL], a.last_enqueued);
+    }
+    const int64_t n = last - first + 1;
+    if (n <= 0 || n > XRING_MAX_W) return;
+    switch ((int)n) {
+#define XRING_CASE(N) case N: xring_sum<N>(a, first); break;
+        XRING_CASE(1) XRING_CASE(2) XRING_CASE(3) XRING_CASE(4) XRING_CASE(5) XRING_CASE(6) XRING_CASE(7) XRING_CASE(8)
+        XRING_CASE(9) XRING_CASE(10) XRING_CASE(11) XRING_CASE(12) XRING_CASE(13) XRING_CASE(14) XRING_CASE(15) XRING_CASE(16)
+#undef XRING_CASE
+    }
+    if (a.k > 0 && blockIdx.x == 0 && threadIdx.x == 0) a.st[T_FLUSHED] = last;
 }
 
 struct sr_args {
diff --git a/stan_amd/csrc/internal.h b/stan_amd/csrc/internal.h
--- a/stan_amd/csrc/internal.h
+++ b/stan_amd/csrc/internal.h
@@ -219,6 +219,11 @@
     int prof_colours = 0;
     int spmv_variant = -1;
     int value_stream_60 = -1;
+    int cg_x_ring = -1;
+    int prof_x_ring_window = 0;
+    int64_t prof_x_ring_flushes = 0;
+    int cg_refresh_60 = -1;
+    int prof_refresh_stream = -1;
     bool profiling = false;
     stan_profile prof{};
     double prof_loads_ms[3] = {0, 0, 0};
diff --git a/stan_amd/csrc/spmv_kernels.inc b/stan_amd/csrc/spmv_kernels.inc
--- a/stan_amd/csrc/spmv_kernels.inc
+++ b/stan_amd/csrc/spmv_kernels.inc
@@ -371,12 +371,21 @@
             x0 *= FX48_INV; x1 *= FX48_INV; xx2 *= FX48_INV;                          \
             u0 *= FX48_INV; u1 *= FX48_INV; u2 *= FX48_INV;                           \
         }                                                                             \
-        y0 += a[0] * x0 + a[1] * x1 + a[2] * xx2;                                     \
-        y1 += a[3] * x0 + a[4] * x1 + a[5] * xx2;                                     \
-        yy2 += a[6] * x0 + a[7] * x1 + a[8] * xx2;                                    \
-        z0 += a[0] * u0 + a[1] * u1 + a[2] * u2;                                      \
-        z1 += a[3] * u0 + a[4] * u1 + a[5] * u2;                                      \
-        z2 += a[6] * u0 + a[7] * u1 + a[8] * u2;                                      \
+        if constexpr (vstream<VT>::P60) {                                             \
+            y0 = s60_row(a[0], a[1], a[2], x0, x1, xx2, y0);                          \
+            y1 = s60_row(a[3], a[4], a[5], x0, x1, xx2, y1);                          \
+            yy2 = s60_row(a[6], a[7], a[8], x0, x1, xx2, yy2);                        \
+            z0 = s60_row(a[0], a[1], a[2], u0, u1, u2, z0);                           \
+            z1 = s60_row(a[3], a[4], a[5], u0, u1, u2, z1);                           \
+            z2 = s60_row(a[6], a[7], a[8], u0, u1, u2, z2);                           \
+        } else {                                                                      \
+            y0 += a[0] * x0 + a[1] * x1 + a[2] * xx2;                                 \
+            y1 += a[3] * x0 + a[4] * x1 + a[5] * xx2;                                 \
+            yy2 += a[6] * x0 + a[7] * x1 + a[8] * xx2;                                \
+            z0 += a[0] * u0 + a[1] * u1 + a[2] * u2;                                  \
+            z1 += a[3] * u0 + a[4] * u1 + a[5] * u2;                                  \
+            z2 += a[6] * u0 + a[7] * u1 + a[8] * u2;                                  \
+        }                                                                             \
     }
         walk_slots<true, 2, vstream<VT>::STRIDE>(cs, cols, slice, lane, k0, k0, k1, vals,
                                                  [&](int64_t c, const VT *vp) { STAN_SPMV2_BLOCK(c, vp) });
diff --git a/stan_amd/csrc/x_ring.h b/stan_amd/csrc/x_ring.h
--- /dev/null
+++ b/stan_amd/csrc/x_ring.h
@@ -0,0 +1,21 @@
+#pragma once
+#include <cstdint>
+
+#if defined(__HIPCC__)
+#define XRING_FN __host__ __device__ __forceinline__
+#else
+#define XRING_FN inline
+#endif
+
+constexpr int XRING_MAX_W = 16;
+
+XRING_FN int xring_window(int64_t rupdate) { return rupdate >= 2 && rupdate <= XRING_MAX_W ? (int)rupdate : 10; }
+
+XRING_FN int xring_slot(int64_t j, int W) { return (int)(j % (W + 1)); }
+
+XRING_FN bool xring_flush_due(int64_t k, int64_t flushed, int W, bool refresh) { return refresh || k - flushed > W; }
+
+XRING_FN int64_t xring_final_iterate(int64_t type, int64_t iters, int64_t xsel, int64_t last_enqueued) {
+    if (type == 0) return last_enqueued;
+    return ((iters ^ xsel) & 1) == 0 ? iters : iters - 1;
+}
diff --git a/stan_amd/hip.py b/stan_amd/hip.py
--- a/stan_amd/hip.py
+++ b/stan_amd/hip.py
@@ -27,6 +27,8 @@
 OPT_CG_REFINE = 20
 OPT_CG_LAZY_SCALING = 21
 OPT_VALUE_STREAM_60 = 22
+OPT_CG_X_RING = 23
+OPT_CG_REFRESH_60 = 24
 VALUE_STREAM_60 = 3
 E_HIP, E_ARG, E_ALLOC, E_DETJ, E_DOF_LAYOUT, E_VALENCE, E_COMM, E_UNSUPPORTED = (
     -1, -2, -3, -4, -5, -6, -7, -8)
@@ -39,7 +41,7 @@
     "stan_hip_ke_hex8_batch", "stan_hip_matrix_to_csr", "stan_hip_spmv", "stan_hip_spmv_bench", "stan_hip_stream_bench",
     "stan_hip_stream60_roundtrip",
     "stan_hip_set_profiling", "stan_hip_get_profile", "stan_hip_set_option", "stan_hip_recover_hex8", "stan_hip_recover_hex8_dev",
-    "stan_hip_nodal_forces_hex8", "stan_hip_pool_info",
+    "stan_hip_nodal_forces_hex8", "stan_hip_pool_info", "stan_hip_cg_loop_info",
     "stan_hip_matrix_plan", "stan_hip_spmv_local", "stan_hip_comm_info", "stan_hip_comm_library",
     "stan_hip_matrix_part_info", "stan_hip_get_profile_rank", "stan_hip_device_info", "stan_hip_matrix_diagonal",
     "stan_hip_recover_hex8_keep", "stan_hip_results_map", "stan_hip_results_free",
@@ -268,6 +270,14 @@
         b, n = C.c_int64(0), C.c_int64(0)
         self._chk(self.lib.stan_hip_pool_info(self.h, C.byref(b), C.byref(n)))
         return b.value, n.value
+
+    def cg_loop_info(self):
+        w, n, s = C.c_int32(0), C.c_int64(0), C.c_int32(-1)
+        self._chk(self.lib.stan_hip_cg_loop_info(self.h, C.byref(w), C.byref(n), C.byref(s)))
+        return w.value, n.value, s.value
+
+    def cg_x_ring_info(self):
+        return self.cg_loop_info()[:2]
 
     def unique_id(self):
         buf = C.create_string_buffer(128)
```
